# KwonGihyun/TweedieMix

Hardware: AMD Instinct MI355X
Metric: denoise steps/sec @ SDXL 1024^2 K=3 concepts (fusion phase); images/sec at 1/2/4/8 GPUs (higher is better)
Workload: dtype bf16

## Files before the change

include/tmix.h:

```cpp
#ifndef TMIX_H
#define TMIX_H

#include <stdint.h>

#ifdef __cplusplus
extern "C" {
#endif

#define TMIX_VERSION 100

enum { TMIX_OK = 0, TMIX_EINVAL = -1, TMIX_ESHAPE = -2, TMIX_EARCH = -3, TMIX_EALIGN = -4 };
enum { TMIX_F32 = 0, TMIX_F16 = 1, TMIX_BF16 = 2 };

int tmix_version(void);
const char* tmix_last_error_string(void);
int tmix_check_device(void);
void tmix_env_refresh(void);

int tmix_prof_begin(uint64_t* slots, int capacity, int detail);
int tmix_prof_end(void);

enum { TMIX_STEP_FUSION = 0, TMIX_STEP_PLAIN = 1, TMIX_STEP_RESAMPLE = 2 };
int tmix_fused_tweedie_step(const float* x, const void* eps, int eps_dtype, const float* masks,
                            float* out_x, float* out_x0, int K, int channels, int64_t hw, int mode,
                            float g, float sa, float s1, float sa_next, float s1_next, int is_last,
                            void* stream);
int tmix_fused_tweedie_step_dev(const float* x, const void* eps, int eps_dtype, const float* masks,
                                int64_t mask_seed_stride, float* out_x, float* out_x0, int K, int channels,
                                int64_t hw, int mode, int rows, int seeds, const float* params, void* stream);
int tmix_fused_tweedie_step_keep_dev(const float* x, const void* eps, int eps_dtype, const float* masks,
                                     int64_t mask_seed_stride, float* out_x, float* out_x0, int K, int channels,
                                     int64_t hw, int mode, int rows, int seeds, const float* params,
                                     const float* keep_x0, int64_t keep_x0_seed_stride, const float* keep_eps,
                                     int64_t keep_eps_seed_stride, const float* keep_w, int64_t keep_w_seed_stride, void* stream);
int tmix_step_prologue(const float* x, float* latent, float* t_dev, const float* params, int seeds, int rows,
                       int64_t n, void* stream);

int tmix_vpred_step(const void* x, const void* v, void* out, int dtype, int64_t n, float g,
                    float sa, float s1, float sa_next, float s1_next, void* stream);
int tmix_video_step_prologue(const float* x, float* x_u, int64_t clip_stride_u, float* t_u, float* x_c, int64_t clip_stride_c,
                             float* t_c, const float* params, int videos, int channels, int frames, int64_t hw, int row_channels,
                             void* stream);
int tmix_vpred_step_dev(float* x, const float* v_u, int64_t clip_stride_u, const float* v_c, int64_t clip_stride_c,
                        const float* params, int videos, int channels, int frames, int64_t hw, void* stream);
int tmix_frame_inject(void* x, int dtype, int clips, int frames, int64_t per_frame, int hard, float interp,
                      float one_minus_interp, void* stream);

enum { TMIX_EPI_NONE = 0, TMIX_EPI_GEGLU = 1, TMIX_EPI_F32OUT = 2 ,
       TMIX_EPI_GELU = 3 ,
       TMIX_EPI_QUICKGELU = 4  };
enum { TMIX_TILE_AUTO = 0, TMIX_TILE_128x128_S2 = 1, TMIX_TILE_256x128_S3 = 2, TMIX_TILE_128x128_S4 = 3,
       TMIX_TILE_256x256_S2 = 4, TMIX_TILE_256x128_W4 = 5, TMIX_TILE_256x256_W4 = 6, TMIX_TILE_128x160_S2 = 7,
       TMIX_TILE_128x160_S2_LW = 8, TMIX_TILE_256x128_S3_LW = 9, TMIX_TILE_128x128_S2_LW = 10, TMIX_TILE_256x256_S2_LW = 11,
       TMIX_TILE_128x160_S4 = 12 ,
       TMIX_TILE_64x160_W5 = 13 ,
       TMIX_TILE_256x320_S2 = 14 ,
       TMIX_TILE_32x160_W5 = 15 ,
       TMIX_TILE_256x256_PH = 16 ,
       TMIX_TILE_256x128_PH = 17,
       TMIX_TILE_128x160_S4_K2 = 18 ,
       TMIX_TILE_128x160_S3_LW = 19 ,
       TMIX_TILE_128x160_S4_LW2 = 20 ,
       TMIX_TILE_128x160_S4_LW4 = 21 ,
       TMIX_TILE_256x320_PH = 22 ,
       TMIX_TILE_128x160_W22 = 23 ,
       TMIX_TILE_CONV_HALO = 26 ,
       TMIX_TILE_COUNT = 26 };
typedef struct {
    const void* A;  int64_t lda, strideA;
    const void* W;  int64_t ldw, strideW;
    void*       C;  int64_t ldc, strideC;
    const float* bias;  int64_t strideBias;
    const void* residual; int64_t ldr, strideR;
    const float* rowgroup_bias;
    int32_t rows_per_group;
    void*   Ct; int64_t ldct, strideCt;
    int32_t n_trans_begin;
    int32_t M, N, K, batch;
    int32_t epilogue;
    int32_t tile_cfg;
    float* row_stats_out; int64_t strideStatsOut, ldStatsOut;
    const float* ln_stats; int64_t strideLnStats, ldLnStats;
    const float* ln_colsum; int64_t strideLnColsum;
    float ln_inv_c, ln_eps;
    int32_t ln_parts, reserved0;
    float* col_stats_out;
    int32_t w_period, reserved1;
} tmix_gemm_desc;
int tmix_gemm_bf16(const tmix_gemm_desc* d, void* stream);
int tmix_gemm_resolve_tile(const tmix_gemm_desc* d, int fp8_operands);
int tmix_gemm_f8copy_tile(int tile_cfg);
int tmix_gemm_prefetch_next(const void* next_weights, int64_t bytes, void* stream);
enum { TMIX_F8_A_BLOCK_SCALES = 1, TMIX_F8_GEGLU_OUT = 2, TMIX_F8_COPY_OUT = 4 };
#define TMIX_COLSTATS_ROWS 32
int tmix_gemm_fp8(const tmix_gemm_desc* d, const uint8_t* scale_a, const uint8_t* scale_w, void* stream);
int tmix_gemm_q_cross_attn(const tmix_gemm_desc* d, const void* K, int64_t ldk, int64_t strideK, const void* Vt, int64_t ldvt, int64_t strideVt,
                           void* O, int64_t ldo, int rows_per_image, int Skv, float scale, void* stream);
int tmix_quantize_fp8_rows(const void* X, int64_t ld, void* Q, int64_t ldq, uint8_t* scale_e8m0, int64_t rows, int K, void* stream);
int tmix_gemm_tile_shape(int tile_cfg, int* bm, int* bn);
int tmix_gemm_stats_parts(int N, int tile_cfg);

enum { TMIX_CONV_S1 = 0, TMIX_CONV_S2 = 1, TMIX_CONV_UP2 = 2, TMIX_CONV_T3 = 3, TMIX_CONV_S2A = 4 };
typedef struct {
    const void* X;
    const void* Wt;
    void*       Y;
    const float* bias;
    const float* batch_bias;
    const void* residual;
    int32_t B, H, W, Cin, Cout, mode;
    int32_t tile_cfg;
    int32_t batch_bias_images;
    float* col_stats_out;
    const void* S1; const void* S2;
    int32_t S1_channels, S2_channels;
} tmix_conv_desc;
int tmix_conv3x3_nhwc(const tmix_conv_desc* d, void* stream);
int tmix_conv3x3_nhwc_fp8(const tmix_conv_desc* d, const uint8_t* scale_x, const uint8_t* scale_w, void* stream);
int tmix_conv_resolve_tile(const tmix_conv_desc* d, int fp8_operands);

int tmix_conv_in(const float* x_nchw, const float* w_ohwi, const float* bias, void* y_nhwc,
                 int B, int Cin, int H, int W, int Cout, void* stream);
int tmix_conv_in_pre(const float* x_nchw, const float* w_ohwi, const float* bias, void* y_nhwc,
                     int B, int Cin, int H, int W, int Cout, const float* pre_w, const float* pre_b, void* stream);
int tmix_conv_out(const void* x_nhwc, const void* w_ohwi, const float* bias, float* y_nchw,
                  int B, int Cin, int H, int W, int Cout, void* stream);

int tmix_attn_fwd(const void* Q, int64_t ldq, int64_t strideQ, const void* K, int64_t ldk, int64_t strideK,
                  const void* Vt, int64_t ldvt, int64_t strideVt, void* O, int64_t ldo, int64_t strideO,
                  int B, int H, int Sq, int Skv, float scale, void* stream);
int tmix_attn_fwd_f8(const void* Q, int64_t ldq, int64_t strideQ, const void* K, int64_t ldk, int64_t strideK,
                     const void* Vt, int64_t ldvt, int64_t strideVt, void* O8, int64_t ldo8, void* scales, int64_t ldScale,
                     int B, int H, int Sq, int Skv, float scale, void* stream);
int64_t tmix_attn_split_ws_bytes(int B, int H, int Sq, int Skv);
int tmix_attn_fwd_ws(const void* Q, int64_t ldq, int64_t strideQ, const void* K, int64_t ldk, int64_t strideK,
                     const void* Vt, int64_t ldvt, int64_t strideVt, void* O, int64_t ldo, int64_t strideO,
                     int B, int H, int Sq, int Skv, float scale, void* ws, int64_t ws_bytes, void* stream);
int tmix_attn_fwd_f8_ws(const void* Q, int64_t ldq, int64_t strideQ, const void* K, int64_t ldk, int64_t strideK,
                        const void* Vt, int64_t ldvt, int64_t strideVt, void* O8, int64_t ldo8, void* scales, int64_t ldScale,
                        int B, int H, int Sq, int Skv, float scale, void* ws, int64_t ws_bytes, void* stream);

int64_t tmix_groupnorm_ws_floats(int B, int C, int groups);
int tmix_groupnorm_ws_chunks(int64_t HW);
int tmix_groupnorm_nhwc(const void* X1, int C1, const void* X2, int C2, void* Y, const float* gamma,
                        const float* beta, float* ws, int B, int64_t HW, int groups, float eps, int silu,
                        void* stream);
int tmix_groupnorm_nhwc_launches(int64_t HW, int C, int groups);
int tmix_groupnorm_nhwc_pre(const void* X1, int C1, const void* X2, int C2, void* Y, const float* gamma,
                            const float* beta, float* ws, int B, int64_t HW, int groups, float eps, int silu,
                            const float* cs1, int cs1_channels, const float* cs2, int cs2_channels, void* stream);
int tmix_groupnorm_nhwc_pre_f8(const void* X1, int C1, const void* X2, int C2, void* Y8, void* scales, const float* gamma,
                               const float* beta, float* ws, int B, int64_t HW, int groups, float eps, int silu,
                               const float* cs1, int cs1_channels, const float* cs2, int cs2_channels, void* stream);
int tmix_layernorm(const void* X, void* Y, const float* gamma, const float* beta, int64_t rows, int C,
                   float eps, void* stream);
int tmix_zero(void* ptr, int64_t nbytes, void* stream);
int tmix_concat_channels(const void* X1, int C1, const void* X2, int C2, void* Y, int64_t rows, void* stream);
int tmix_timestep_embedding(const float* values, float* out, int count, int dim, void* stream);
int tmix_softmax_rows(const float* S, int64_t ld_s, void* P, int64_t ld_p, int64_t rows, int cols, float scale, void* stream);
int tmix_softmax_rows_causal(const float* S, int64_t ld_s, void* P, int64_t ld_p, int64_t rows, int cols, float scale,
                             int seq, void* stream);
int tmix_softmax_rows_masked(const float* S, int64_t ld_s, void* P, int64_t ld_p, int64_t rows, int cols, int valid, float scale,
                             void* stream);
int tmix_temporal_attn(const void* QKV, int64_t ld, void* O, int64_t ldo, int clips, int frames, int64_t hw, int heads,
                       float scale, void* stream);
int tmix_lora_down(void* A, int64_t lda, int K, int64_t rows, const void* D, int P, int nsets, const float* dcolsum, const float* dbias,
                   float eps, const int* sets, int64_t rows_per_set, void* stream);
int tmix_affine_clamp(const float* x, float* y, int64_t n, float scale, float shift, float lo, float hi, void* stream);
int tmix_linear_small(const float* in, const void* W, const float* bias, const float* add, float* out,
                      int M, int N, int K, int act_in, int act_out, void* stream);
int tmix_linear_small_sections(const float* in, const void* W, const float* bias, float* out, int M, int N, int K,
                               int act_in, const int* sec_starts, int nsec, void* stream);

int tmix_conv3x3_f32(const float* x_nchw, const float* w_oihw, const float* bias, float* y_nchw, int B, int Cin, int H, int W, int Cout,
                     int stride, int silu, void* stream);
int tmix_adaptive_avgpool_f32(const float* x, float* y, int64_t planes, int H, int W, int OH, int OW, void* stream);
int tmix_linear_f32(const float* in, const float* W, const float* bias, float* out, int M, int N, int K, int act_in, int act_out, void* stream);
int tmix_i2v_temporal_encoder(const float* x, float* y, int clips, int frames, int channels, int64_t hw, const float* ln_gamma, const float* ln_beta,
                              const float* wq, const float* wk, const float* wv, const float* wo, const float* bo,
                              const float* w1, const float* b1, const float* w2, const float* b2, void* stream);

int tmix_xattn_token_maps(const void* Q, int64_t ldq, int64_t strideQ, const void* K, int64_t ldk, int64_t strideK, float* maps,
                          int B, int H, int Sq, int Lk, int row0, int row_step, int n_rows, const int32_t* tokens, int n_tok,
                          int accumulate, float scale, void* stream);

// ... 5 lines not shown
```

tweediemix_amd/csrc/gemm_conv.hip:

```cpp
#include "gemm_kernel.h"
#include "gemm_tilings.h"
#include <stdlib.h>

using namespace tmix_gemm;

namespace tmix_gemm {

bool f8_lockstep(int tile_cfg, int K, bool f8out) {
    return tile_cfg >= 1 && tile_cfg <= NUM_CFG && tile_has(tile_cfg, CAP_F8_LOCKSTEP) && K % 128 == 0 && !f8out;
}

int f8copy_tile(int tile_cfg) {
    if (tile_cfg < 1 || tile_cfg > NUM_CFG) TMIX_FAIL(TMIX_EINVAL, "gemm_f8copy_tile: tile_cfg=%d", tile_cfg);
    int cfg = TILINGS[tile_cfg].runs_as;
    while (!tile_has(cfg, CAP_F8C)) cfg = TILINGS[cfg].fb;
    return cfg;
}

#define TMIX_REFUSE(code, ...) do { tmix_set_error(__VA_ARGS__); return TileChoice{0, 0, (code)}; } while (0)

TileChoice resolve_tile(const TileTraits& t, int cfg) {
    const bool staged = t.n_trans_begin < 0 && (t.epilogue == TMIX_EPI_GEGLU ? (t.wide & 2) : (t.wide & 1));
    if (cfg <= 0 || cfg > NUM_CFG)
        cfg = (int64_t)((t.M + 255) / 256) * ((t.N + 127) / 128) * t.batch >= 192 ? 2 : 1;
// ... 144 lines not shown
        if (d->reserved0 & TMIX_F8_GEGLU_OUT) {
            if (d->epilogue != TMIX_EPI_GEGLU || !d->Ct || d->ldct < (int64_t)d->batch * d->M || (d->ldc % 8) || (d->strideC % 8) || (((uintptr_t)d->C) & 7))
                TMIX_FAIL(TMIX_EINVAL, "gemm_fp8: e4m3 GEGLU output needs the GEGLU epilogue, Ct = scale buffer [N/64][ldct >= batch*M] and 8-byte aligned C rows");
            p.f8out = 1; p.scale_out = (unsigned char*)d->Ct; p.ldScaleOut = d->ldct;
        }
    } else if (d->reserved0 & ~TMIX_F8_COPY_OUT) TMIX_FAIL(TMIX_EINVAL, "gemm: the fp8 operand flags in reserved0 belong to tmix_gemm_fp8");
    if (d->reserved0 & TMIX_F8_COPY_OUT) {
        if (has_trans || d->epilogue != TMIX_EPI_NONE || (d->reserved0 & TMIX_F8_GEGLU_OUT) || !d->Ct || (d->M % 32) || (d->N % 32) || (d->ldct % 8) || d->ldct < d->N
            || (((uintptr_t)d->Ct) & 7) || d->strideCt < (int64_t)d->batch * d->M * d->ldct)
            TMIX_FAIL(TMIX_EINVAL, "gemm: the e4m3 copy needs the plain bf16 epilogue, M %% 32 == 0, N %% 32 == 0, Ct = bytes [batch*M][ldct >= N, %% 8 == 0] and strideCt = byte offset of the scale array behind them");
        p.f8copy = (unsigned char*)d->Ct; p.ldF8copy = d->ldct;
        p.scale_out = (unsigned char*)d->Ct + d->strideCt; p.ldScaleOut = (int64_t)d->batch * d->M;
    }
    if (d->row_stats_out && (has_trans || d->epilogue != TMIX_EPI_NONE)) TMIX_FAIL(TMIX_EINVAL, "gemm: row_stats_out needs the plain bf16 epilogue");
    if (d->row_stats_out && (d->tile_cfg < 1 || d->tile_cfg > NUM_CFG || (((uintptr_t)d->row_stats_out) & 7) || (d->strideStatsOut & 1) || d->ldStatsOut < d->M))
        TMIX_FAIL(TMIX_EINVAL, "gemm: row_stats_out needs an explicit tile_cfg (its partial count depends on it) and 8-byte alignment");
    if (d->ln_stats && (!d->ln_colsum || !(d->ln_inv_c > 0.f) || d->ln_parts < 1 || d->ln_parts > 16 || (int64_t)d->ln_parts * d->ldLnStats * 8 >= (1ll << 31) || (((uintptr_t)d->ln_stats) & 7) || (d->strideLnStats & 1) || d->ldLnStats < d->M))
        TMIX_FAIL(TMIX_EINVAL, "gemm: fused LayerNorm needs ln_colsum, ln_inv_c > 0, 1 <= ln_parts <= 16 and 8-byte aligned ln_stats (< 2 GiB)");
    p.stats_out = d->row_stats_out; p.strideStatsOut = d->strideStatsOut; p.ldStatsOut = d->ldStatsOut;
    p.ln_stats = d->ln_stats; p.strideLnStats = d->strideLnStats; p.ldLnStats = d->ldLnStats; p.ln_parts = d->ln_parts;
    p.ln_colsum = d->ln_colsum; p.strideLnColsum = d->strideLnColsum; p.ln_inv_c = d->ln_inv_c; p.ln_eps = d->ln_eps;
    const bool c16 = d->C && aligned16(d->C) && (d->ldc % 8) == 0 && (d->strideC % 8) == 0;
    const bool r16 = !d->residual || (aligned16(d->residual) && (d->ldr % 8) == 0 && (d->strideR % 8) == 0);
    p.wide = 0;
    if (!tmix_env(TMIX_ENV_NARROW_EPILOGUE)) {
        if (d->epilogue == TMIX_EPI_GEGLU) { if (c16 || p.f8out) p.wide |= 2; }
        else if (d->epilogue == TMIX_EPI_F32OUT) { if (aligned16(d->C) && (d->ldc % 4) == 0 && (d->strideC % 4) == 0 && (d->N % 8) == 0) p.wide |= 1; }
        else if (c16 && r16 && (d->N % 8) == 0) p.wide |= 1;
        if (has_trans && aligned16(d->Ct) && (d->ldct % 8) == 0 && (d->strideCt % 8) == 0) p.wide |= 4;
    }
    if (d->col_stats_out) {
        if (fp8) TMIX_FAIL(TMIX_EINVAL, "gemm_fp8: col_stats_out is compiled for the bf16 tilings only (the fp8 loop would be remapped to a bf16 kernel over e4m3 bytes)");
        if (has_trans || d->epilogue != TMIX_EPI_NONE || d->row_stats_out || (d->reserved0 & TMIX_F8_COPY_OUT) || d->batch != 1 || (d->M % TMIX_COLSTATS_ROWS) || (d->N % 8)
            || !aligned16(d->col_stats_out) || !(p.wide & 1))
            TMIX_FAIL(TMIX_EINVAL, "gemm: col_stats_out needs the plain staged bf16 epilogue (16-byte aligned C / residual rows, N %% 8 == 0), batch == 1, M %% 32 == 0, "
                                   "and neither row_stats_out nor the e4m3 copy");
        p.cs_out = d->col_stats_out;
    }
    if (p.f8out && !(p.wide & 2)) TMIX_FAIL(TMIX_EINVAL, "gemm_fp8: e4m3 GEGLU output needs the staged epilogue");
    if (p.f8copy && !(p.wide & 1)) TMIX_FAIL(TMIX_EALIGN, "gemm: the e4m3 copy needs the staged epilogue (16-byte aligned C / residual rows, N %% 8 == 0)");
    if (fp8 && has_trans && !(p.wide & 4)) TMIX_FAIL(TMIX_EALIGN, "gemm_fp8: the transposed region needs a 16-byte aligned Ct with ldct %% 8 == 0");
    return TMIX_OK;
}

static int gemm_entry(const tmix_gemm_desc* d, bool fp8, const uint8_t* scaleA, const uint8_t* scaleW, void* stream, const QAExtra* qa = nullptr) {
    Params p;
    if (const int rc = gemm_params(d, fp8, scaleA, scaleW, qa != nullptr, p)) return rc;
    if (qa) return launch_qattn(p, *qa, d->batch, (hipStream_t)stream);
    return launch(0, p, d->batch, d->tile_cfg, (hipStream_t)stream);
}

alignas(16) static const uint8_t NO_SCALES[16] = {};

extern "C" int tmix_gemm_resolve_tile(const tmix_gemm_desc* d, int fp8_operands) {
    Params p;
    if (const int rc = gemm_params(d, fp8_operands != 0, fp8_operands ? NO_SCALES : nullptr, fp8_operands ? NO_SCALES : nullptr, false, p)) return rc;
    const TileChoice r = resolve_tile(traits_of(0, p, d->batch), d->tile_cfg);
    return r.err ? r.err : r.cfg;
}

extern "C" int tmix_gemm_q_cross_attn(const tmix_gemm_desc* d, const void* K, int64_t ldk, int64_t strideK, const void* Vt, int64_t ldvt, int64_t strideVt,
                                      void* O, int64_t ldo, int rows_per_image, int Skv, float scale, void* stream) {
    if (!d) TMIX_FAIL(TMIX_EINVAL, "gemm_q_cross_attn: null descriptor");
    if (d->reserved0 || d->residual || d->row_stats_out || d->col_stats_out || d->rowgroup_bias || d->epilogue != TMIX_EPI_NONE || (d->n_trans_begin >= 0 && d->n_trans_begin < d->N))
        TMIX_FAIL(TMIX_EINVAL, "gemm_q_cross_attn: the projection takes a bias and a folded LayerNorm only");
    const QAExtra x = {K, ldk, strideK, Vt, ldvt, strideVt, O, ldo, rows_per_image, Skv, scale};
    return gemm_entry(d, false, nullptr, nullptr, stream, &x);
}

extern "C" int tmix_gemm_bf16(const tmix_gemm_desc* d, void* stream) { return gemm_entry(d, false, nullptr, nullptr, stream); }

extern "C" int tmix_gemm_fp8(const tmix_gemm_desc* d, const uint8_t* scale_a, const uint8_t* scale_w, void* stream) {
    return gemm_entry(d, true, scale_a, scale_w, stream);
}

static int conv_params(const tmix_conv_desc* d, const uint8_t* scale_x, const uint8_t* scale_w, Params& p) {
    const bool fp8 = scale_x != nullptr;
    if (!d || !d->X || !d->Wt || !d->Y) TMIX_FAIL(TMIX_EINVAL, "conv3x3: null descriptor/operand");
    if (fp8 && (!scale_w || (d->Cin % 128) || d->S1 || d->S2 || (((uintptr_t)scale_x) & 3)))
        TMIX_FAIL(TMIX_EINVAL, "conv3x3_fp8: needs both scale arrays (scale_x 4-byte aligned), Cin %% 128 == 0 and no shortcut taps");
    if (d->B <= 0 || d->H <= 0 || d->W <= 0 || d->Cin <= 0 || d->Cout <= 0) TMIX_FAIL(TMIX_ESHAPE, "conv3x3: empty problem");
    if (d->Cin % BK) TMIX_FAIL(TMIX_ESHAPE, "conv3x3: Cin=%d must be a multiple of %d", d->Cin, BK);
    if (d->Cout % 4) TMIX_FAIL(TMIX_ESHAPE, "conv3x3: Cout=%d must be a multiple of 4", d->Cout);
    if (d->mode < TMIX_CONV_S1 || d->mode > TMIX_CONV_S2A) TMIX_FAIL(TMIX_EINVAL, "conv3x3: bad mode %d", d->mode);
    if ((d->mode == TMIX_CONV_S2 || d->mode == TMIX_CONV_S2A) && ((d->H | d->W) & 1)) TMIX_FAIL(TMIX_ESHAPE, "conv3x3: stride-2 needs even H,W");
    if (!aligned16(d->X) || !aligned16(d->Wt) || (((uintptr_t)d->Y) & 7)) TMIX_FAIL(TMIX_EALIGN, "conv3x3: pointer alignment");
    if ((d->bias && (((uintptr_t)d->bias) & 15)) || (d->batch_bias && (((uintptr_t)d->batch_bias) & 15))) TMIX_FAIL(TMIX_EALIGN, "conv3x3: bias alignment");
    p = {};
    p.H = d->H; p.Wd = d->W; p.Cin = d->Cin; p.mode = d->mode;
    p.ntaps = d->mode == TMIX_CONV_T3 ? 3 : 9;
    const bool half = d->mode == TMIX_CONV_S2 || d->mode == TMIX_CONV_S2A;
    p.Ho = half ? d->H / 2 : (d->mode == TMIX_CONV_UP2 ? d->H * 2 : d->H);
    p.Wo = half ? d->W / 2 : (d->mode == TMIX_CONV_UP2 ? d->W * 2 : d->W);
    const int64_t M = (int64_t)d->B * p.Ho * p.Wo;
    if (M > 0x7fffffff / 4) TMIX_FAIL(TMIX_ESHAPE, "conv3x3: too many output pixels");
    if ((int64_t)d->B * d->H * d->W * d->Cin >= (1ll << 30) || (int64_t)d->Cout * 9 * d->Cin >= (1ll << 30)) TMIX_FAIL(TMIX_ESHAPE, "conv3x3: operand larger than 2 GiB");
    p.A = (const bf16_t*)d->X;
    p.W = (const bf16_t*)d->Wt; p.ldw = p.ntaps * (int64_t)d->Cin;
    p.C = (bf16_t*)d->Y; p.ldc = d->Cout;
    p.bias = d->bias;
    p.R = (const bf16_t*)d->residual; p.ldr = d->Cout;
    p.rgb = d->batch_bias; p.rows_per_group = p.Ho * p.Wo * (d->batch_bias_images > 1 ? d->batch_bias_images : 1);
    p.n_trans_begin = -1;
    p.M = (int)M; p.N = d->Cout; p.K = p.ntaps * d->Cin;
    if (d->S1 || d->S2) {
        const int c1 = d->S1_channels, c2 = d->S2 ? d->S2_channels : 0;
        if (!d->S1 || d->mode != TMIX_CONV_S1 || c1 <= 0 || (c1 % BK) || c2 < 0 || (c2 % BK) || (d->S2 && c2 == 0) || !aligned16(d->S1) || (d->S2 && !aligned16(d->S2)) || d->residual)
            TMIX_FAIL(TMIX_EINVAL, "conv3x3: shortcut taps need the stride-1 mode, S1 (S2 only with S1), channel counts that are multiples of %d, 16-byte alignment and no residual", BK);
        if ((int64_t)d->B * d->H * d->W * (c1 > c2 ? c1 : c2) >= (1ll << 30) || (int64_t)d->Cout * (9ll * d->Cin + c1 + c2) >= (1ll << 30)) TMIX_FAIL(TMIX_ESHAPE, "conv3x3: shortcut operand larger than 2 GiB");
        p.S1 = (const bf16_t*)d->S1; p.S2 = (const bf16_t*)d->S2; p.c1s = c1; p.c2s = c2;
        p.bytesS1 = (unsigned)((int64_t)d->B * d->H * d->W * c1 * 2); p.bytesS2 = (unsigned)((int64_t)d->B * d->H * d->W * c2 * 2);
        p.K += c1 + c2;
        p.ldw = p.K;
    }
    p.epilogue = TMIX_EPI_NONE;
    p.bytesA = (unsigned)((int64_t)d->B * d->H * d->W * d->Cin * (fp8 ? 1 : 2));
    p.bytesW = (unsigned)((int64_t)d->Cout * p.K * (fp8 ? 1 : 2));
    if (fp8) { p.scaleA = scale_x; p.scaleW = scale_w; p.ldScaleA = d->Cin / 32; }
    p.wide = (!tmix_env(TMIX_ENV_NARROW_EPILOGUE) && aligned16(d->Y) && (d->Cout % 8) == 0 && (!d->residual || aligned16(d->residual))) ? 1 : 0;
    if (p.S1 && !p.wide) TMIX_FAIL(TMIX_EALIGN, "conv3x3: shortcut taps need the staged epilogue (16-byte aligned Y, Cout %% 8 == 0)");
    if (d->col_stats_out) {
        if ((M % TMIX_COLSTATS_ROWS) || !aligned16(d->col_stats_out) || !p.wide)
            TMIX_FAIL(TMIX_EINVAL, "conv3x3: col_stats_out needs B*Ho*Wo %% 32 == 0, Cout %% 8 == 0 and 16-byte aligned Y / residual");
        p.cs_out = d->col_stats_out;
    }
    return TMIX_OK;
}

static int conv_entry(const tmix_conv_desc* d, const uint8_t* scale_x, const uint8_t* scale_w, void* stream) {
    Params p;
    if (const int rc = conv_params(d, scale_x, scale_w, p)) return rc;
    return launch(1, p, 1, d->tile_cfg, (hipStream_t)stream);
}

extern "C" int tmix_conv_resolve_tile(const tmix_conv_desc* d, int fp8_operands) {
    Params p;
    if (const int rc = conv_params(d, fp8_operands ? NO_SCALES : nullptr, fp8_operands ? NO_SCALES : nullptr, p)) return rc;
    const TileChoice r = resolve_tile(traits_of(1, p, 1), d->tile_cfg);
    return r.err ? r.err : r.cfg;
}

extern "C" int tmix_conv3x3_nhwc(const tmix_conv_desc* d, void* stream) { return conv_entry(d, nullptr, nullptr, stream); }

extern "C" int tmix_conv3x3_nhwc_fp8(const tmix_conv_desc* d, const uint8_t* scale_x, const uint8_t* scale_w, void* stream) {
    if (!scale_x) TMIX_FAIL(TMIX_EINVAL, "conv3x3_fp8: null scale array");
    return conv_entry(d, scale_x, scale_w, stream);
}
```

tweediemix_amd/csrc/gemm_kernel.h:

```cpp
#pragma once
#include "common.h"
#include <type_traits>
#include <stdlib.h>

namespace tmix_gemm {

#ifndef TMIX_ABL
#define TMIX_ABL 0
#endif
constexpr int ABL = TMIX_ABL;

constexpr int BK = 64;
typedef __attribute__((ext_vector_type(8))) __bf16 frag_ab;

static __device__ __forceinline__ float xor32_sum(float x) {
    auto r = __builtin_amdgcn_permlane32_swap(__float_as_uint(x), __float_as_uint(x), false, false);
    return __uint_as_float(r[0]) + __uint_as_float(r[1]);
}

static __device__ __forceinline__ float quad_max(float x) {
    float y = __int_as_float(__builtin_amdgcn_update_dpp(0, __float_as_int(x), 0xB1, 0xf, 0xf, false));
    x = fmaxf(x, y);
    y = __int_as_float(__builtin_amdgcn_update_dpp(0, __float_as_int(x), 0x4E, 0xf, 0xf, false));
    return fmaxf(x, y);
}

template <int CTRL> static __device__ __forceinline__ float dpp_row(float x) {
    return __int_as_float(__builtin_amdgcn_update_dpp(0, __float_as_int(x), CTRL, 0xf, 0xf, false));
}
static __device__ __forceinline__ float swap32_sum(float a, float b) {
    auto r = __builtin_amdgcn_permlane32_swap(__float_as_uint(a), __float_as_uint(b), false, false);
    return __uint_as_float(r[0]) + __uint_as_float(r[1]);
}
static __device__ __forceinline__ float swap16_sum(float a, float b) {
    auto r = __builtin_amdgcn_permlane16_swap(__float_as_uint(a), __float_as_uint(b), false, false);
    return __uint_as_float(r[0]) + __uint_as_float(r[1]);
}

struct Params {
    const bf16_t* A; int64_t lda, strideA;
    const bf16_t* W; int64_t ldw, strideW;
    bf16_t* C; int64_t ldc, strideC;
    const float* bias; int64_t strideBias;
    const bf16_t* R; int64_t ldr, strideR;
    const float* rgb; int rows_per_group;
    bf16_t* Ct; int64_t ldct, strideCt; int n_trans_begin;
    int M, N, K, tiles_m, tiles_n, group_m, epilogue;
    unsigned bytesA, bytesW;
    float* stats_out; int64_t strideStatsOut, ldStatsOut;
    const float* ln_stats; int64_t strideLnStats, ldLnStats; const float* ln_colsum; int64_t strideLnColsum;
    float ln_inv_c, ln_eps; int ln_parts;
    int H, Wd, Cin, Ho, Wo, mode, ntaps;
    unsigned long long* prof; int prof_detail;
    int wide;
    const unsigned char* scaleA; const unsigned char* scaleW; int64_t strideScaleA, strideScaleW;
    int64_t ldScaleA;
    unsigned char* scale_out; int64_t ldScaleOut; int f8out;
    unsigned char* f8copy; int64_t ldF8copy;
    const char* pf; long long pf_bytes;
    int pf_per;
    int w_period, w_groups; unsigned w_magic;
    float* cs_out;
    const bf16_t* S1; const bf16_t* S2; int c1s, c2s; unsigned bytesS1, bytesS2;
};

static __device__ __forceinline__ void blds16(__amdgpu_buffer_rsrc_t rsrc, unsigned voff, unsigned soff, char* lds_dst) {
    __builtin_amdgcn_raw_ptr_buffer_load_lds(rsrc, (__attribute__((address_space(3))) void*)lds_dst, 16, voff, soff, 0, 0);
}

constexpr int f8_block_cap(int bn) { return bn >= 256 ? 88 : 224; }

template <int N> static __device__ __forceinline__ void wait_vmcnt() { asm volatile("s_waitcnt vmcnt(%0)" ::"n"(N) : "memory"); }

template <int BM, int BN, int WM, int WN, int NS, int CONV, int LW = 0, int PH = 0, int KS = 1, int CS = 0, int EK = 0, int SC = 0>
__global__ void __launch_bounds__((WM * WN * KS + LW) * 64, LW ? (NS * (BM + BN) * 128 > 80 * 1024 ? 2 : 3) : (KS == 1 && WM * WN == 4 && NS * (BM + BN) * 128 > 80 * 1024) ? 1 : 2)
gemm_conv_kernel(const Params p) {
    constexpr bool PHL = PH >= 1 && PH <= 3;
    static_assert(!PHL || (WM * WN == 8 && !LW && !CONV && NS == 4 && BM % 128 == 0 && BN % 32 == 0 && (BM / WM) % 32 == 0 && (BN / WN) % 32 == 0), "phase-offset mainloop geometry");
    static_assert(PH <= 3 || KS == 1, "fp8 lock-step loop: no in-workgroup split-K");
    static_assert(!(CONV && PH >= 4) || (PH == 5 && !SC && BM % ((LW ? LW : WM * WN)) == 0 && BM / (LW ? LW : WM * WN) <= 64), "fp8 convolution geometry");
    static_assert(KS == 1 || (KS == 2 && !LW && !PH && !CONV), "in-workgroup split-K geometry");
    static_assert(!SC || (CONV && (LW == 0 || LW == 2)), "shortcut taps belong to the convolution (lock-step tilings, with or without two loader waves)");
    constexpr bool F8C = !CONV && (LW ? (PH >= 4 && EK == 4) : true) && (BM / WM / 32) * (BN / WN / 32) <= 8;
    constexpr bool F8 = PH >= 2;
    constexpr bool F8B = PH == 3 || PH == 5;
    constexpr bool F8L = PH >= 4;
    constexpr int SCP = (F8L && F8B) ? 1 : 0;
    constexpr int EB = F8 ? 1 : 2;
    constexpr int NW = WM * WN;
    constexpr int TM = BM / WM, TN = BN / WN;
    constexpr int FM = TM / 32, FN = TN / 32;
    constexpr int A_TILE = BM * 128, B_TILE = BN * 128, STAGE = A_TILE + B_TILE + SCP * 1024;
    static_assert(!SCP || 4 * BM <= 1024, "scale piece");
    constexpr int SLOT = (BM + BN) * 64;
    constexpr int RING = PHL ? 4 * SLOT : NS * STAGE;
    constexpr int SW = LW ? LW : NW * KS;
    constexpr int IA = BM / 8, IB = BN / 8;
    constexpr int RA = (IA + SW - 1) / SW, RB = (IB + SW - 1) / SW;
    constexpr int L = RA + RB + SCP;
    static_assert(RA >= 1 && RB >= 1 && FM >= 1 && FN >= 1, "tile/wave geometry");
    static_assert(PHL || (NS - 2) * L <= 63, "vmcnt immediate");

    extern __shared__ __attribute__((aligned(16))) char smem[];
#ifndef TMIX_NO_KERNARG_TOUCH
    kernarg_touch<(int)sizeof(Params)>();
#endif
    const int tid = threadIdx.x;
    const int lane = tid & 63;
    const int w = __builtin_amdgcn_readfirstlane(tid >> 6);
    const int kg = KS > 1 ? w / NW : 0;
    const int wm_ = KS > 1 ? w - kg * NW : w;
    const int wr = wm_ / WN, wc = wm_ - wr * WN;
    const bool prof_on = p.prof != nullptr && tid == 0;
    unsigned long long pt0 = 0, pt1 = 0, pt2 = 0;
    if (prof_on) pt0 = prof_enter(p.prof, (blockIdx.x | blockIdx.y) == 0, p.prof_detail);
    constexpr int PFU = 8;
    unsigned pf_keep[PFU];
#pragma unroll
    for (int u = 0; u < PFU; ++u) pf_keep[u] = 0;
    if (p.pf && (!LW || w >= WM * WN)) {
        const long long nwg = (long long)gridDim.x * gridDim.y, nth = (LW ? LW : WM * WN * KS) * 64;
        const long long lines = (p.pf_bytes + 127) >> 7; const int per = p.pf_per;
        const long long first = ((long long)blockIdx.y * gridDim.x + blockIdx.x) * nth + (LW ? tid - WM * WN * 64 : tid);
#pragma unroll
        for (int u = 0; u < PFU; ++u) {
            const long long ln = first + (long long)u * nwg * nth;
            if (u < per && ln < lines) asm volatile("global_load_dword %0, %1, off" : "=v"(pf_keep[u]) : "v"(p.pf + (ln << 7)) : "memory");
        }
    }
    const bool loader = LW && (w >= NW);
    const bool stager = LW ? loader : true;
    const int sw_id = LW ? max(w - NW, 0) : w;

#ifdef TMIX_XCD_X_ONLY
    const int bid = xcd_remap(blockIdx.x, gridDim.x), by = blockIdx.y;
#else
    int bid, by;
    xcd_remap_grid(bid, by);
#endif
    const int per_group = p.group_m * p.tiles_n;
    const int grp = bid / per_group;
    const int first_m = grp * p.group_m;
    const int gsize = min(p.tiles_m - first_m, p.group_m);
    const int rem = bid - grp * per_group;
    const int tile_n = rem / gsize, tile_m = first_m + (rem - tile_n * gsize);
    const int m0 = tile_m * BM, n0 = tile_n * BN;
    const int m0l = (ABL & 1) ? 0 : m0, n0l = (ABL & 1) ? 0 : n0;
    const int bzw = p.w_period > 0 ? (int)__umulhi((unsigned)by, p.w_magic) : by;
    const int bz = p.w_period > 0 ? (by - bzw * p.w_groups) * p.w_period + bzw : by;

    const bf16_t* Ab = (const bf16_t*)((const char*)p.A + (int64_t)bz * p.strideA * EB);
    const bf16_t* Wb = (const bf16_t*)((const char*)p.W + (int64_t)bzw * p.strideW * EB);
    const __amdgpu_buffer_rsrc_t rsA = __builtin_amdgcn_make_buffer_rsrc((void*)Ab, 0, p.bytesA, 0x00020000);
    const __amdgpu_buffer_rsrc_t rsW = __builtin_amdgcn_make_buffer_rsrc((void*)Wb, 0, p.bytesW, 0x00020000);

    const int lrow = lane >> 3;
    auto slot_a = [&](int r) { int i = r * SW + sw_id; if constexpr (IA % SW != 0) i = min(i, IA - 1); return i; };
    auto slot_w = [&](int r) { int i = r * SW + sw_id; if constexpr (IB % SW != 0) i = min(i, IB - 1); return i; };
    constexpr int RAa = (LW && !CONV) ? 1 : RA, RBa = LW ? 1 : RB;
    unsigned woff[RBa], aoff[RAa];
    int asw[(CONV && !LW) ? RA : 1];
    unsigned cbase[CONV ? RA : 1], cmask[CONV ? RA : 1];
    int cpix[(CONV && SC) ? RA : 1];
    auto conv_row = [&](int r, int m, unsigned swb) __attribute__((always_inline)) {
        if constexpr (CONV) {
            const int hw = p.Ho * p.Wo;
            const int b = m / hw, rem = m - b * hw;
            const int py = rem / p.Wo, px = rem - py * p.Wo;
            int iy0, ix0; unsigned par = 0;
            if (p.mode == TMIX_CONV_S1 || p.mode == TMIX_CONV_T3) { iy0 = py - 1; ix0 = px - 1; }
            else if (p.mode == TMIX_CONV_S2) { iy0 = 2 * py - 1; ix0 = 2 * px - 1; }
            else if (p.mode == TMIX_CONV_S2A) { iy0 = 2 * py; ix0 = 2 * px; }
            else { iy0 = (py - 1) >> 1; ix0 = (px - 1) >> 1; par = (unsigned)((py - 1) & 1) << 16 | (unsigned)((px - 1) & 1) << 17; }
            unsigned mk = 0;
#pragma unroll
            for (int t = 0; t < 9; ++t) {
                if (t >= p.ntaps) break;
                const int ky = p.mode == TMIX_CONV_T3 ? t : t / 3, kx = p.mode == TMIX_CONV_T3 ? 1 : t - (t / 3) * 3;
                bool ok;
                if (p.mode == TMIX_CONV_UP2) { const int uy = py + ky - 1, ux = px + kx - 1; ok = (uy >= 0) & (uy < 2 * p.H) & (ux >= 0) & (ux < 2 * p.Wd); }
                else { const int iy = iy0 + ky, ix = ix0 + kx; ok = (iy >= 0) & (iy < p.H) & (ix >= 0) & (ix < p.Wd); }
                mk |= (unsigned)ok << t;
            }
            cbase[r] = (unsigned)(((b * p.H + iy0) * p.Wd + ix0) * p.Cin) * (unsigned)EB + swb;
            cmask[r] = mk | par;
            if constexpr (SC) cpix[r] = (b * p.H + py) * p.Wd + px;
        }
    };
    unsigned aoffp[2], amaxp[2], woffp[2], wmaxp[2], swp[2];
    if constexpr (LW) {
        if (loader) {
#pragma unroll
            for (int pp = 0; pp < 2; ++pp) {
                const int par = (LW >= 2) ? (sw_id & 1) : pp;
                const unsigned sw = ((lane & 7) ^ ((4 * par + (lane >> 4)) & 7)) * 8;
                swp[pp] = sw;
                woffp[pp] = (unsigned)(n0l + par * 8 + lrow) * (unsigned)p.ldw * (unsigned)EB + sw * 2u;
                wmaxp[pp] = (unsigned)(p.N - 1) * (unsigned)p.ldw * (unsigned)EB + sw * 2u;
                aoffp[pp] = (unsigned)(m0l + par * 8 + lrow) * (unsigned)p.lda * (unsigned)EB + sw * 2u;
                amaxp[pp] = (unsigned)(p.M - 1) * (unsigned)p.lda * (unsigned)EB + sw * 2u;
            }
            if constexpr (CONV) {
#pragma unroll
                for (int r = 0; r < RA; ++r) {
                    int m = m0l + slot_a(r) * 8 + lrow; if (m > p.M - 1) m = p.M - 1;
                    conv_row(r, m, swp[r & 1] * 2u);
                }
            }
        }
    } else
    if (stager && !PHL) {
#pragma unroll
    for (int r = 0; r < RB; ++r) {
        const int idx = slot_w(r);
        const int sw = ((lane & 7) ^ ((4 * idx + (lane >> 4)) & 7)) * 8;
        int n = n0l + idx * 8 + lrow; if (n > p.N - 1) n = p.N - 1;
        woff[r] = (unsigned)n * (unsigned)p.ldw * (unsigned)EB + (unsigned)sw * 2u;
    }
#pragma unroll
    for (int r = 0; r < RA; ++r) {
        const int idx = slot_a(r);
        const int sw = ((lane & 7) ^ ((4 * idx + (lane >> 4)) & 7)) * 8;
        int m = m0l + idx * 8 + lrow; if (m > p.M - 1) m = p.M - 1;
        asw[r] = sw;
        if constexpr (CONV) {
            conv_row(r, m, (unsigned)sw * 2u);
            aoff[r] = 0;
        } else {
            aoff[r] = (unsigned)m * (unsigned)p.lda * (unsigned)EB + (unsigned)sw * 2u;
        }
    }
    }

    constexpr int PA = PHL ? BM / 16 / NW : 1, PB = PHL ? (BN / 16 + NW - 1) / NW : 1;
    auto ph_w = [&](int r) { int i = r * NW + w; if constexpr ((BN / 16) % NW != 0) i = min(i, BN / 16 - 1); return i; };
    unsigned phA[PA], phW[PB];
    if constexpr (PHL) {
        const unsigned ch = (unsigned)(((lane & 3) ^ ((lane >> 4) & 3)) * (16 / EB));
#pragma unroll
        for (int r = 0; r < PA; ++r) {
            int m = m0l + (r * NW + w) * 16 + (lane >> 2); if (m > p.M - 1) m = p.M - 1;
            phA[r] = ((unsigned)m * (unsigned)p.lda + ch) * (unsigned)EB;
        }
#pragma unroll
        for (int r = 0; r < PB; ++r) {
            int n = n0l + ph_w(r) * 16 + (lane >> 2); if (n > p.N - 1) n = p.N - 1;
            phW[r] = ((unsigned)n * (unsigned)p.ldw + ch) * (unsigned)EB;
        }
    }
    auto ph_stage = [&](int slot, int s) {
        char* sA = smem + slot * SLOT;
        char* sW = sA + BM * 64;
#pragma unroll
        for (int r = 0; r < PA; ++r) blds16(rsA, phA[r], (unsigned)s * 64u, sA + (r * NW + w) * 1024);
#pragma unroll
        for (int r = 0; r < PB; ++r) blds16(rsW, phW[r], (unsigned)s * 64u, sW + ph_w(r) * 1024);
    };

    const int nk = p.K / (F8L ? 2 * BK : BK);
    int tap = 0, cc = 0;
    int cpt = CONV ? p.Cin / (F8L ? 2 * BK : BK) : 1;
    const int ntaps_all = SC ? p.ntaps + (p.c1s > 0) + (p.c2s > 0) : p.ntaps;

    unsigned cvo[RA];
    constexpr int SRW = (CONV && SCP) ? BM / SW : 1;
    int sb_ = 0, sy_ = 0, sx_ = 0; unsigned scv = 0x80000000u;
    if constexpr (CONV && SCP) {
        if (stager) {
            const int hw = p.Ho * p.Wo;
            int m = m0l + sw_id * SRW + min(lane, SRW - 1); if (m > p.M - 1) m = p.M - 1;
            sb_ = m / hw; const int rem = m - sb_ * hw;
            sy_ = rem / p.Wo; sx_ = rem - sy_ * p.Wo;
        }
    }
    auto conv_tap_offsets = [&]() __attribute__((always_inline)) {
        if constexpr (SC) {
            if (tap >= p.ntaps) {
                const int Cs = tap == p.ntaps ? p.c1s : p.c2s;
#pragma unroll
                for (int r = 0; r < RA; ++r)
                    cvo[r] = (unsigned)(cpix[r] * Cs + (LW ? (int)swp[r & 1] : asw[LW ? 0 : r])) * 2u;
                cpt = Cs / BK;
                return;
            }
        }
        const int ky = p.mode == TMIX_CONV_T3 ? tap : tap / 3, kx = p.mode == TMIX_CONV_T3 ? 1 : tap - ky * 3;
        const unsigned pixb = (unsigned)p.Cin * (unsigned)EB, rowb = (unsigned)p.Wd * pixb;
        if (p.mode == TMIX_CONV_UP2) {
            const unsigned sd = (ky == 2 ? rowb : 0u) + (kx == 2 ? pixb : 0u), ay = ky == 1 ? rowb : 0u, ax = kx == 1 ? pixb : 0u;
#pragma unroll
            for (int r = 0; r < RA; ++r) {
                const unsigned o = cbase[r] + sd + ((cmask[r] >> 16) & 1u) * ay + ((cmask[r] >> 17) & 1u) * ax;
                cvo[r] = ((cmask[r] >> tap) & 1u) ? o : 0x80000000u;
            }
        } else {
            const unsigned sd = (unsigned)ky * rowb + (unsigned)kx * pixb;
#pragma unroll
            for (int r = 0; r < RA; ++r) cvo[r] = ((cmask[r] >> tap) & 1u) ? cbase[r] + sd : 0x80000000u;
        }
        if constexpr (CONV && SCP) {
            int iy, ix; bool ok;
            if (p.mode == TMIX_CONV_S1 || p.mode == TMIX_CONV_T3) { iy = sy_ + ky - 1;     ix = sx_ + kx - 1;     ok = (iy >= 0) & (iy < p.H) & (ix >= 0) & (ix < p.Wd); }
            else if (p.mode == TMIX_CONV_S2) { iy = 2 * sy_ + ky - 1; ix = 2 * sx_ + kx - 1; ok = (iy >= 0) & (iy < p.H) & (ix >= 0) & (ix < p.Wd); }
            else if (p.mode == TMIX_CONV_S2A) { iy = 2 * sy_ + ky; ix = 2 * sx_ + kx; ok = (iy < p.H) & (ix < p.Wd); }
            else { const int uy = sy_ + ky - 1, ux = sx_ + kx - 1;
                   ok = (uy >= 0) & (uy < 2 * p.H) & (ux >= 0) & (ux < 2 * p.Wd); iy = uy >> 1; ix = ux >> 1; }
            scv = ok ? (unsigned)((sb_ * p.H + iy) * p.Wd + ix) * (unsigned)(p.Cin / 32) : 0x80000000u;
        }
    };
    if constexpr (CONV) { if (stager) conv_tap_offsets(); }

    const bool sc_mine = SCP && (CONV ? lane < SRW : (lane % SW == sw_id) && (16 * lane < 4 * BM));
    unsigned sc_voff = 0;
    __amdgpu_buffer_rsrc_t rsSc = rsA;
    if constexpr (SCP) {
        if constexpr (CONV) rsSc = __builtin_amdgcn_make_buffer_rsrc((void*)p.scaleA, 0, (int)(p.bytesA / 32), 0x00020000);
        else {
            rsSc = __builtin_amdgcn_make_buffer_rsrc((void*)p.scaleA, 0, (int)((int64_t)(p.K / 32) * p.ldScaleA), 0x00020000);
            sc_voff = (unsigned)((16 * lane) / BM) * (unsigned)p.ldScaleA + (unsigned)((16 * lane) % BM) + (unsigned)(bz * p.strideScaleA + m0l);
        }
    }
    auto scale_piece = [&](char* sA, int kt) __attribute__((always_inline)) {
        if constexpr (SCP && CONV) {
            if (sc_mine) __builtin_amdgcn_raw_ptr_buffer_load_lds(rsSc, (__attribute__((address_space(3))) void*)(sA + A_TILE + B_TILE + sw_id * SRW * 4), 4, scv, (unsigned)cc * 4u, 0, 0);
        } else if constexpr (SCP) { if (sc_mine) blds16(rsSc, sc_voff, (unsigned)kt * 4u * (unsigned)p.ldScaleA, sA + A_TILE + B_TILE); }
    };
    auto dma_piece = [&](const int r, char* sA, int kt) __attribute__((always_inline)) {
        if constexpr (!CONV && !LW) {
            if (r < RA) blds16(rsA, aoff[r], (unsigned)kt * (BK * 2), sA + slot_a(r) * 1024);
            else if (r < RA + RB) blds16(rsW, woff[r - RA], (unsigned)kt * (BK * 2), sA + A_TILE + slot_w(r - RA) * 1024);
            else scale_piece(sA, kt);
        }
    };
    auto stage = [&](int buf, int kt) __attribute__((always_inline)) {
        char* sA = smem + buf * STAGE;
        char* sW = sA + A_TILE;
        bool a_done = false;
        unsigned wk = (unsigned)kt * (BK * 2);
#ifndef TMIX_ABL_WSEQ
        if constexpr (CONV && !LW) {
            const int tap_u = __builtin_amdgcn_readfirstlane(tap), cc_u = __builtin_amdgcn_readfirstlane(cc);
            if (SC && tap_u >= p.ntaps) wk = (unsigned)(p.ntaps * p.Cin + (tap_u > p.ntaps ? p.c1s : 0)) * 2u + (unsigned)cc_u * (BK * 2);
            else wk = (unsigned)(tap_u * p.Cin) * (unsigned)EB + (unsigned)cc_u * (BK * 2);
        }
#endif
        if constexpr (CONV && SC) {
            const int tap_u = __builtin_amdgcn_readfirstlane(tap);
            const void* base = tap_u < p.ntaps ? (const void*)Ab : (tap_u == p.ntaps ? (const void*)p.S1 : (const void*)p.S2);
            const unsigned bytes = tap_u < p.ntaps ? p.bytesA : (tap_u == p.ntaps ? p.bytesS1 : p.bytesS2);
            const __amdgpu_buffer_rsrc_t rs = __builtin_amdgcn_make_buffer_rsrc((void*)base, 0, bytes, 0x00020000);
            a_done = true;
#pragma unroll
            for (int r = 0; r < RA; ++r) blds16(rs, cvo[r], (unsigned)cc * (BK * 2), sA + slot_a(r) * 1024);
        }
        if (!a_done)
#pragma unroll
        for (int r = 0; r < RA; ++r) {
            if constexpr (CONV) blds16(rsA, cvo[r], (unsigned)cc * (BK * 2), sA + slot_a(r) * 1024);
            else if constexpr (LW) blds16(rsA, min(aoffp[(r * LW) & 1] + (unsigned)(slot_a(r) >> 1) * (unsigned)(16 * EB * p.lda), amaxp[(r * LW) & 1]),
                                          (unsigned)kt * (BK * 2), sA + slot_a(r) * 1024);
            else                blds16(rsA, aoff[r], (unsigned)kt * (BK * 2), sA + slot_a(r) * 1024);
        }
#pragma unroll
        for (int r = 0; r < RB; ++r) {
            if constexpr (LW) blds16(rsW, min(woffp[(r * LW) & 1] + (unsigned)(slot_w(r) >> 1) * (unsigned)(16 * EB * p.ldw), wmaxp[(r * LW) & 1]),
                                     wk, sW + slot_w(r) * 1024);
            else              blds16(rsW, woff[r], wk, sW + slot_w(r) * 1024);
        }
        scale_piece(sA, kt);
// ... 481 lines not shown
                    if (m + 8 <= p.M) *(uint4*)dst = v;
                    else {
                        const unsigned u[4] = {v.x, v.y, v.z, v.w};
                        for (int k = 0; k < 8 && m + k < p.M; ++k) dst[k] = (bf16_t)(u[k >> 1] >> ((k & 1) * 16));
                    }
                }
            }
            if (prof_on) prof_leave(p.prof, p.prof_detail, pt0, pt1, pt2);
            return;
        }
        if constexpr (SQ) {
            bf16_t* Ct = p.Ct + (int64_t)bz * p.strideCt;
            if (EK == 3 || (p.wide & 4)) {
                constexpr int CF = (FN % 2 == 0) ? 2 : 1, SR = CF * 64 + 16, LPR = CF * 4, RPI = 64 / LPR, NP = 32 / RPI;
                char* stg = smem + w * STG_MAX;
                const int rr = lane / LPR, cc = (lane % LPR) * 8;
#pragma unroll
                for (int i = 0; i < FM; ++i) {
                    const int nl = n0 + wc * TN + i * 32 + l31;
                    const float bv = (bias && nl < p.N) ? bias[nl] : 0.f;
#pragma unroll
                    for (int c = 0; c < FN / CF; ++c) {
#pragma unroll
                        for (int jj = 0; jj < CF; ++jj)
#pragma unroll
                            for (int g = 0; g < 4; ++g) {
                                const int j = c * CF + jj, ml = wr * TM + j * 32 + g * 8 + lhi * 4;
                                const float4 rs = p.ln_stats ? *(const float4*)(ln_rs + ml) : make_float4(1.f, 1.f, 1.f, 1.f);
                                uint2 v;
                                v.x = pack_bf2(fmaf(acc[i][j][g * 4 + 0], rs.x, bv), fmaf(acc[i][j][g * 4 + 1], rs.y, bv));
                                v.y = pack_bf2(fmaf(acc[i][j][g * 4 + 2], rs.z, bv), fmaf(acc[i][j][g * 4 + 3], rs.w, bv));
                                *(uint2*)(stg + l31 * SR + (jj * 32 + g * 8 + lhi * 4) * 2) = v;
                            }
#pragma unroll
                        for (int ps = 0; ps < NP; ++ps) {
                            const int r = ps * RPI + rr, n = n0 + wc * TN + i * 32 + r, m = m0 + wr * TM + c * CF * 32 + cc;
                            const uint4 v = *(const uint4*)(stg + r * SR + cc * 2);
                            if (n >= p.N || m >= p.M) continue;
                            bf16_t* dst = Ct + (int64_t)(n - p.n_trans_begin) * p.ldct + m;
                            if (m + 8 <= p.M) *(uint4*)dst = v;
                            else {
                                const unsigned u[4] = {v.x, v.y, v.z, v.w};
                                for (int k = 0; k < 8 && m + k < p.M; ++k) dst[k] = (bf16_t)(u[k >> 1] >> ((k & 1) * 16));
                            }
                        }
                    }
                }
                if (prof_on) prof_leave(p.prof, p.prof_detail, pt0, pt1, pt2);
                return;
            }
#pragma unroll
            for (int i = 0; i < FM; ++i) {
                const int n = n0 + wc * TN + i * 32 + l31;
                if (n >= p.N) continue;
                const float bv = bias ? bias[n] : 0.f;
                bf16_t* row = Ct + (int64_t)(n - p.n_trans_begin) * p.ldct;
#pragma unroll
                for (int j = 0; j < FN; ++j)
#pragma unroll
                    for (int g = 0; g < 4; ++g) {
                        const int ml = wr * TM + j * 32 + g * 8 + lhi * 4, m = m0 + ml;
                        if (m >= p.M) continue;
                        const float4 rs = p.ln_stats ? *(const float4*)(ln_rs + ml) : make_float4(1.f, 1.f, 1.f, 1.f);
                        const float o0 = fmaf(acc[i][j][g * 4 + 0], rs.x, bv), o1 = fmaf(acc[i][j][g * 4 + 1], rs.y, bv);
                        const float o2 = fmaf(acc[i][j][g * 4 + 2], rs.z, bv), o3 = fmaf(acc[i][j][g * 4 + 3], rs.w, bv);
                        if (m + 3 < p.M && ((p.ldct & 3) == 0)) {
                            uint2 v;
                            v.x = pack_bf2(o0, o1);
                            v.y = pack_bf2(o2, o3);
                            *(uint2*)(row + m) = v;
                        } else {
                            const float o[4] = {o0, o1, o2, o3};
#pragma unroll
                            for (int r = 0; r < 4; ++r) if (m + r < p.M) row[m + r] = f2bf(o[r]);
                        }
                    }
            }
        }
        if (prof_on) prof_leave(p.prof, p.prof_detail, pt0, pt1, pt2);
        return;
    }

    bf16_t* Cb = p.C + (int64_t)bz * p.strideC;
    if (EK == 1 || (EK == 0 && p.epilogue == TMIX_EPI_GEGLU)) {
        if (EK == 1 || (p.wide & 2)) {
            char* stg = smem + w * STG_MAX;
            auto chunk = [&](int i, int j0, auto cf_tag) {
                constexpr int CF = decltype(cf_tag)::value, OC = CF * 16, SR = OC * 2 + 16, LPR = OC / 8, RPI = 64 / LPR, NP = 32 / RPI;
                const int rr = lane / LPR, cc = (lane % LPR) * 8;
#pragma unroll
                for (int jj = 0; jj < CF; ++jj) {
                    const int j = j0 + jj;
#pragma unroll
                    for (int g = 0; g < 2; ++g) {
                        float o[4];
                        const float4 ba = *(const float4*)(bias_lds + wc * TN + j * 32 + g * 8 + lhi * 4), bg = *(const float4*)(bias_lds + wc * TN + j * 32 + g * 8 + lhi * 4 + 16);
                        const float bav[4] = {ba.x, ba.y, ba.z, ba.w}, bgv[4] = {bg.x, bg.y, bg.z, bg.w};
#pragma unroll
                        for (int r = 0; r < 4; ++r) {
                            const float a = fmaf(acc[i][j][g * 4 + r], rs_row[i], bav[r]), gt = fmaf(acc[i][j][(g + 2) * 4 + r], rs_row[i], bgv[r]);
                            o[r] = a * gelu_erf_f(gt);
                        }
                        uint2 v; v.x = pack_bf2(o[0], o[1]); v.y = pack_bf2(o[2], o[3]);
                        *(uint2*)(stg + l31 * SR + (jj * 16 + g * 8 + lhi * 4) * 2) = v;
                    }
                }
#pragma unroll
                for (int ps = 0; ps < NP; ++ps) {
                    const int r = ps * RPI + rr, m = m0 + wr * TM + i * 32 + r;
                    const uint4 v = *(const uint4*)(stg + r * SR + cc * 2);
                    const int nb = n0 + wc * TN + (j0 + cc / 16) * 32;
                    const int col = (n0 + wc * TN) / 2 + j0 * 16 + cc;
                    if constexpr (CF >= 2) {
                        if (p.f8out) {
                            const unsigned u[4] = {v.x, v.y, v.z, v.w};
                            float f[8], am = 0.f;
#pragma unroll
                            for (int k = 0; k < 4; ++k) { f[2 * k] = __uint_as_float(u[k] << 16); f[2 * k + 1] = __uint_as_float(u[k] & 0xffff0000u);
                                                          am = fmaxf(am, fmaxf(fabsf(f[2 * k]), fabsf(f[2 * k + 1]))); }
                            am = quad_max(am);
                            const int e = e8m0_for_amax(am);
                            const float inv = exp2_neg_int(e);
                            int q0 = __builtin_amdgcn_cvt_pk_fp8_f32(f[0] * inv, f[1] * inv, 0, false); q0 = __builtin_amdgcn_cvt_pk_fp8_f32(f[2] * inv, f[3] * inv, q0, true);
                            int q1 = __builtin_amdgcn_cvt_pk_fp8_f32(f[4] * inv, f[5] * inv, 0, false); q1 = __builtin_amdgcn_cvt_pk_fp8_f32(f[6] * inv, f[7] * inv, q1, true);
                            if (m >= p.M || nb >= p.N) continue;
                            *(uint2*)((unsigned char*)p.C + (int64_t)bz * p.strideC + (int64_t)m * p.ldc + col) = make_uint2((unsigned)q0, (unsigned)q1);
                            if ((lane & 3) == 0) p.scale_out[(int64_t)(col >> 5) * p.ldScaleOut + (int64_t)bz * p.M + m] = (unsigned char)(e + 127);
                            continue;
                        }
                    }
                    if (m >= p.M || nb >= p.N) continue;
                    *(uint4*)(Cb + (int64_t)m * p.ldc + col) = v;
                }
            };
#pragma unroll
            for (int i = 0; i < FM; ++i) {
                constexpr int C4 = FN / 4, R4 = FN % 4;
#pragma unroll
                for (int c = 0; c < C4; ++c) chunk(i, c * 4, std::integral_constant<int, 4>{});
                if constexpr (R4 >= 2) chunk(i, C4 * 4, std::integral_constant<int, 2>{});
                if constexpr (R4 & 1) chunk(i, FN - 1, std::integral_constant<int, 1>{});
            }
            if (prof_on) prof_leave(p.prof, p.prof_detail, pt0, pt1, pt2);
            return;
        }
#pragma unroll
        for (int i = 0; i < FM; ++i) {
            const int m = m0 + wr * TM + i * 32 + l31;
            if (m >= p.M) continue;
#pragma unroll
            for (int j = 0; j < FN; ++j) {
                const int nb = n0 + wc * TN + j * 32;
                if (nb >= p.N) continue;
#pragma unroll
                for (int g = 0; g < 2; ++g) {
                    const int nv = nb + g * 8 + lhi * 4;
                    float o[4];
#pragma unroll
                    for (int r = 0; r < 4; ++r) {
                        float a = acc[i][j][g * 4 + r], gt = acc[i][j][(g + 2) * 4 + r];
                        if (bias) { a = fmaf(a, rs_row[i], bias[nv + r]); gt = fmaf(gt, rs_row[i], bias[nv + 16 + r]); }
                        else { a *= rs_row[i]; gt *= rs_row[i]; }
                        o[r] = a * gelu_erf_f(gt);
                    }
                    uint2 v; v.x = pack_bf2(o[0], o[1]); v.y = pack_bf2(o[2], o[3]);
                    *(uint2*)(Cb + (int64_t)m * p.ldc + nb / 2 + g * 8 + lhi * 4) = v;
// ... 12 lines not shown
#pragma unroll
        for (int i = 0; i < FM; ++i) {
#pragma unroll
            for (int q = 0; q < 4; ++q) { sa1[i][q] = 0.f; sa2[i][q] = 0.f; }
            sb1[i][0] = sb1[i][1] = sb2[i][0] = sb2[i][1] = 0.f;
        }
        auto cs_flush = [&](float (&cv)[16], int mb, int nc, bool ncok, auto cf_tag) __attribute__((always_inline)) {
            constexpr int CF = decltype(cf_tag)::value;
            float t[8], u[4];
#pragma unroll
            for (int k = 0; k < 8; ++k) t[k] = swap32_sum(cv[k], cv[8 + k]);
#pragma unroll
            for (int k = 0; k < 4; ++k) u[k] = swap16_sum(t[k], t[k + 4]);
#pragma unroll
            for (int k = 0; k < 4; ++k) u[k] += dpp_row<0x128>(u[k]);
            if constexpr (CF == 1) {
#pragma unroll
                for (int k = 0; k < 4; ++k) u[k] += dpp_row<0x124>(u[k]);
            }
            if (!(lane & (CF == 1 ? 12 : 8)) && mb < p.M && ncok)
                *(float4*)(p.cs_out + ((int64_t)(mb >> 5) * 2 + (lane >> 5)) * p.N + nc + ((lane >> 4) & 1) * 4) = make_float4(u[0], u[1], u[2], u[3]);
        };
        auto cs_add = [&](float (&cv)[16], const uint4& v) __attribute__((always_inline)) {
            const unsigned u[4] = {v.x, v.y, v.z, v.w};
#pragma unroll
            for (int k = 0; k < 4; ++k) {
                const float lo = __uint_as_float(u[k] << 16), hi = __uint_as_float(u[k] & 0xffff0000u);
                cv[2 * k] += lo; cv[2 * k + 1] += hi;
                cv[8 + 2 * k] = fmaf(lo, lo, cv[8 + 2 * k]); cv[9 + 2 * k] = fmaf(hi, hi, cv[9 + 2 * k]);
            }
        };
        auto chunk = [&](int j0, auto cf_tag, auto fl_tag) __attribute__((always_inline)) {
            constexpr int CF = decltype(cf_tag)::value, CW = CF * 32, SR = CW * 4 + 16, LPR = CW / 8, RPI = 64 / LPR, NP = 32 / RPI;
            constexpr int FL = decltype(fl_tag)::value;
            const int rr = lane / LPR, cc = (lane % LPR) * 8;
            const int nc = n0 + wc * TN + j0 * 32 + cc;
            const bool ncok = nc < p.N;
            if constexpr ((FL & 1) != 0) {
                constexpr int CI = CF == 2 ? 0 : (FN / 2) * 4;
                const bool lnf = p.ln_stats != nullptr;
                const float4 bq0 = *(const float4*)(bias_lds + wc * TN + j0 * 32 + cc), bq1 = *(const float4*)(bias_lds + wc * TN + j0 * 32 + cc + 4);
                const float bq[8] = {bq0.x, bq0.y, bq0.z, bq0.w, bq1.x, bq1.y, bq1.z, bq1.w};
                float tq[8];
                if constexpr (CONV) {
                    const float4 t0 = *(const float4*)(rgb_lds + wc * TN + j0 * 32 + cc), t1 = *(const float4*)(rgb_lds + wc * TN + j0 * 32 + cc + 4);
                    tq[0] = t0.x; tq[1] = t0.y; tq[2] = t0.z; tq[3] = t0.w; tq[4] = t1.x; tq[5] = t1.y; tq[6] = t1.z; tq[7] = t1.w;
                }
#pragma unroll
                for (int i = 0; i < FM; ++i) {
                    const int mb = m0 + wr * TM + i * 32;
                    float cv[(FL & 8) ? 16 : 1];
                    if constexpr ((FL & 8) != 0) {
#pragma unroll
                        for (int k = 0; k < 16; ++k) cv[k] = 0.f;
                    }
#pragma unroll
                    for (int jj = 0; jj < CF; ++jj)
#pragma unroll
                        for (int g = 0; g < 4; ++g)
                            *(float4*)(stg + l31 * SR + (jj * 32 + g * 8 + lhi * 4) * 4) =
                                make_float4(acc[i][j0 + jj][g * 4 + 0], acc[i][j0 + jj][g * 4 + 1], acc[i][j0 + jj][g * 4 + 2], acc[i][j0 + jj][g * 4 + 3]);
#pragma unroll
                    for (int ps = 0; ps < NP; ++ps) {
                        const int r = ps * RPI + rr, m = mb + r;
                        const float4 v0 = *(const float4*)(stg + r * SR + cc * 4), v1 = *(const float4*)(stg + r * SR + cc * 4 + 16);
                        const float rsl = ln_rs[wr * TM + i * 32 + r];
                        const float rs = lnf ? rsl : 1.f;
                        float o[8] = {v0.x, v0.y, v0.z, v0.w, v1.x, v1.y, v1.z, v1.w};
#pragma unroll
                        for (int k = 0; k < 8; ++k) o[k] = fmaf(o[k], rs, bq[k]);
                        if constexpr (CONV) {
#pragma unroll
                            for (int k = 0; k < 8; ++k) o[k] += tq[k];
                        }
                        if constexpr (WPREF) {
                            const uint4 rq = rw[i * WP_I + CI + (CF == 2 ? (j0 / 2) * 4 : 0) + ps];
                            const unsigned ru[4] = {rq.x, rq.y, rq.z, rq.w};
#pragma unroll
                            for (int k = 0; k < 4; ++k) { o[2 * k] += __uint_as_float(ru[k] << 16); o[2 * k + 1] += __uint_as_float(ru[k] & 0xffff0000u); }
                        }
                        uint4 v;
                        v.x = pack_bf2(o[0], o[1]); v.y = pack_bf2(o[2], o[3]); v.z = pack_bf2(o[4], o[5]); v.w = pack_bf2(o[6], o[7]);
                        const bool ok = m < p.M && ncok;
                        if (ok) *(uint4*)(Cb + (int64_t)m * p.ldc + nc) = v;
                        if constexpr (F8C && (FL & 4) != 0) {
                            const unsigned u8[4] = {v.x, v.y, v.z, v.w};
                            float f[8], am = 0.f;
#pragma unroll
                            for (int k = 0; k < 4; ++k) { f[2 * k] = __uint_as_float(u8[k] << 16); f[2 * k + 1] = __uint_as_float(u8[k] & 0xffff0000u);
                                                          am = fmaxf(am, fmaxf(fabsf(f[2 * k]), fabsf(f[2 * k + 1]))); }
                            am = quad_max(am);
                            const int e = e8m0_for_amax(am);
                            const float inv = exp2_neg_int(e);
                            int q0 = __builtin_amdgcn_cvt_pk_fp8_f32(f[0] * inv, f[1] * inv, 0, false); q0 = __builtin_amdgcn_cvt_pk_fp8_f32(f[2] * inv, f[3] * inv, q0, true);
                            int q1 = __builtin_amdgcn_cvt_pk_fp8_f32(f[4] * inv, f[5] * inv, 0, false); q1 = __builtin_amdgcn_cvt_pk_fp8_f32(f[6] * inv, f[7] * inv, q1, true);
                            if (ok) {
                                *(uint2*)(p.f8copy + ((int64_t)bz * p.M + m) * p.ldF8copy + nc) = make_uint2((unsigned)q0, (unsigned)q1);
                                if ((lane & 3) == 0) p.scale_out[(int64_t)(nc >> 5) * p.ldScaleOut + (int64_t)bz * p.M + m] = (unsigned char)(e + 127);
                            }
                        }
                        if constexpr ((FL & 2) != 0) {
                            const unsigned u[4] = {v.x, v.y, v.z, v.w};
                            float a1 = 0.f, a2 = 0.f;
#pragma unroll
                            for (int k = 0; k < 4; ++k) {
                                const float lo = __uint_as_float(u[k] << 16), hi = __uint_as_float(u[k] & 0xffff0000u);
                                a1 += lo + hi; a2 = fmaf(lo, lo, a2); a2 = fmaf(hi, hi, a2);
                            }
                            if (!ok) { a1 = 0.f; a2 = 0.f; }
                            if constexpr (CF == 2) { sa1[i][ps] += a1; sa2[i][ps] += a2; } else { sb1[i][ps] += a1; sb2[i][ps] += a2; }
                        }
                        if constexpr ((FL & 8) != 0) cs_add(cv, v);
                    }
                    if constexpr ((FL & 8) != 0) cs_flush(cv, mb, nc, ncok, cf_tag);
                }
                return;
            }
            float bv[8];
#pragma unroll
            for (int k = 0; k < 8; ++k) bv[k] = 0.f;
            if (bias && ncok && !(ABL & 16)) {
                const float4 b0 = *(const float4*)(bias + nc), b1 = *(const float4*)(bias + nc + 4);
                bv[0] = b0.x; bv[1] = b0.y; bv[2] = b0.z; bv[3] = b0.w; bv[4] = b1.x; bv[5] = b1.y; bv[6] = b1.z; bv[7] = b1.w;
            }
#pragma unroll
            for (int i = 0; i < FM; ++i) {
                const int mb = m0 + wr * TM + i * 32;
                float cv[(FL & 8) ? 16 : 1];
                if constexpr ((FL & 8) != 0) {
#pragma unroll
                    for (int k = 0; k < 16; ++k) cv[k] = 0.f;
                }
                uint4 rv[NP];
                if (Rb && !(ABL & 64)) {
#pragma unroll
                    for (int ps = 0; ps < NP; ++ps) {
                        const int m = mb + ps * RPI + rr;
                        if constexpr (WPREF) rv[ps] = rw[i * WP_I + (CF == 2 ? (j0 / 2) * 4 : (FN / 2) * 4) + ps];
                        else if (m < p.M && ncok) rv[ps] = *(const uint4*)(Rb + (int64_t)m * p.ldr + nc);
                    }
                }
#pragma unroll
                for (int jj = 0; jj < CF; ++jj)
#pragma unroll
                    for (int g = 0; g < 4; ++g)
                        *(float4*)(stg + l31 * SR + (jj * 32 + g * 8 + lhi * 4) * 4) =
                            make_float4(acc[i][j0 + jj][g * 4 + 0], acc[i][j0 + jj][g * 4 + 1], acc[i][j0 + jj][g * 4 + 2], acc[i][j0 + jj][g * 4 + 3]);
#pragma unroll
                for (int ps = 0; ps < NP; ++ps) {
                    const int r = ps * RPI + rr, m = mb + r;
                    const float4 v0 = *(const float4*)(stg + r * SR + cc * 4), v1 = *(const float4*)(stg + r * SR + cc * 4 + 16);
                    if (m >= p.M || !ncok) continue;
                    float o[8] = {v0.x, v0.y, v0.z, v0.w, v1.x, v1.y, v1.z, v1.w};
                    if (bias) { const float rs = p.ln_stats ? ln_rs[wr * TM + i * 32 + r] : 1.f;
#pragma unroll
                                for (int k = 0; k < 8; ++k) o[k] = fmaf(o[k], rs, bv[k]); }
                    else if (p.ln_stats) { const float rs = ln_rs[wr * TM + i * 32 + r];
#pragma unroll
                                for (int k = 0; k < 8; ++k) o[k] *= rs; }
                    if (p.rgb) {
                        const float* rg = p.rgb + (int64_t)(m / p.rows_per_group) * p.N + nc;
                        const float4 b0 = *(const float4*)rg, b1 = *(const float4*)(rg + 4);
                        o[0] += b0.x; o[1] += b0.y; o[2] += b0.z; o[3] += b0.w; o[4] += b1.x; o[5] += b1.y; o[6] += b1.z; o[7] += b1.w;
                    }
                    if (p.epilogue == TMIX_EPI_GELU) {
#pragma unroll
                        for (int k = 0; k < 8; ++k) o[k] = gelu_erf_f(o[k]);
                    } else if (p.epilogue == TMIX_EPI_QUICKGELU) {
#pragma unroll
                        for (int k = 0; k < 8; ++k) o[k] = o[k] * __builtin_amdgcn_rcpf(1.0f + __builtin_amdgcn_exp2f(-2.4554669595930157f * o[k]));
                    }
                    if (Rb && !(ABL & 64)) {
                        const unsigned u[4] = {rv[ps].x, rv[ps].y, rv[ps].z, rv[ps].w};
#pragma unroll
                        for (int k = 0; k < 4; ++k) { o[2 * k] += bf2f((bf16_t)(u[k] & 0xffff)); o[2 * k + 1] += bf2f((bf16_t)(u[k] >> 16)); }
                    }
                    if (f32out) {
                        float* dst = (float*)p.C + (int64_t)bz * p.strideC + (int64_t)m * p.ldc + nc;
                        *(float4*)dst = make_float4(o[0], o[1], o[2], o[3]);
                        *(float4*)(dst + 4) = make_float4(o[4], o[5], o[6], o[7]);
                    } else {
                        uint4 v;
                        v.x = pack_bf2(o[0], o[1]); v.y = pack_bf2(o[2], o[3]); v.z = pack_bf2(o[4], o[5]); v.w = pack_bf2(o[6], o[7]);
                        if constexpr (ABL & 32) asm volatile("" :: "v"(v.x), "v"(v.y), "v"(v.z), "v"(v.w));
                        else *(uint4*)(Cb + (int64_t)m * p.ldc + nc) = v;
                        if constexpr (F8C) if (p.f8copy) {
                            const unsigned u8[4] = {v.x, v.y, v.z, v.w};
                            float f[8], am = 0.f;
#pragma unroll
                            for (int k = 0; k < 4; ++k) { f[2 * k] = __uint_as_float(u8[k] << 16); f[2 * k + 1] = __uint_as_float(u8[k] & 0xffff0000u);
                                                          am = fmaxf(am, fmaxf(fabsf(f[2 * k]), fabsf(f[2 * k + 1]))); }
                            am = quad_max(am);
                            const int e = e8m0_for_amax(am);
                            const float inv = exp2_neg_int(e);
                            int q0 = __builtin_amdgcn_cvt_pk_fp8_f32(f[0] * inv, f[1] * inv, 0, false); q0 = __builtin_amdgcn_cvt_pk_fp8_f32(f[2] * inv, f[3] * inv, q0, true);
                            int q1 = __builtin_amdgcn_cvt_pk_fp8_f32(f[4] * inv, f[5] * inv, 0, false); q1 = __builtin_amdgcn_cvt_pk_fp8_f32(f[6] * inv, f[7] * inv, q1, true);
                            *(uint2*)(p.f8copy + ((int64_t)bz * p.M + m) * p.ldF8copy + nc) = make_uint2((unsigned)q0, (unsigned)q1);
                            if ((lane & 3) == 0) p.scale_out[(int64_t)(nc >> 5) * p.ldScaleOut + (int64_t)bz * p.M + m] = (unsigned char)(e + 127);
                        }
                        if (sto) {
                            const unsigned u[4] = {v.x, v.y, v.z, v.w};
                            float a1 = 0.f, a2 = 0.f;
#pragma unroll
                            for (int k = 0; k < 4; ++k) {
                                const float lo = __uint_as_float(u[k] << 16), hi = __uint_as_float(u[k] & 0xffff0000u);
                                a1 += lo + hi; a2 = fmaf(lo, lo, a2); a2 = fmaf(hi, hi, a2);
                            }
                            if constexpr (CF == 2) { sa1[i][ps] += a1; sa2[i][ps] += a2; } else { sb1[i][ps] += a1; sb2[i][ps] += a2; }
                        }
                        if constexpr ((FL & 8) != 0) cs_add(cv, v);
                    }
                }
                if constexpr ((FL & 8) != 0) cs_flush(cv, mb, nc, ncok, cf_tag);
            }
        };
        constexpr int C2 = FN / 2;
        auto chunks = [&](auto fl_tag) __attribute__((always_inline)) {
#pragma unroll
            for (int c = 0; c < C2; ++c) chunk(c * 2, std::integral_constant<int, 2>{}, fl_tag);
            if constexpr (FN & 1) chunk(FN - 1, std::integral_constant<int, 1>{}, fl_tag);
        };
        const bool fastp = (WPREF || !Rb) && !f32out && p.epilogue == TMIX_EPI_NONE && (!p.rgb || (CONV && rgb_one)) && !(ABL & 0xf0);
        bool f8q = false;
        if constexpr (F8C) f8q = p.f8copy != nullptr;
        if constexpr (EK == 4) { if constexpr (F8C) { if (!sto) chunks(std::integral_constant<int, 5>{}); else chunks(std::integral_constant<int, 7>{}); } }
        else if constexpr (CS) { if (!fastp) chunks(std::integral_constant<int, 8>{}); else chunks(std::integral_constant<int, 9>{}); }
        else if (!fastp) chunks(std::integral_constant<int, 0>{});
        else if (!f8q) { if (!sto) chunks(std::integral_constant<int, 1>{}); else chunks(std::integral_constant<int, 3>{}); }
        else { if constexpr (F8C) { if (!sto) chunks(std::integral_constant<int, 5>{}); else chunks(std::integral_constant<int, 7>{}); } }
        if (sto) {
#pragma unroll
            for (int i = 0; i < FM; ++i) {
                if constexpr (C2 > 0) {
#pragma unroll
                    for (int q = 0; q < 4; ++q) {
                        float a1 = sa1[i][q], a2 = sa2[i][q];
#pragma unroll
                        for (int off = 1; off < 8; off <<= 1) { a1 += __shfl_xor(a1, off); a2 += __shfl_xor(a2, off); }
                        if ((lane & 7) == 0) redw[wc * BM + wr * TM + i * 32 + q * 8 + (lane >> 3)] = make_float2(a1, a2);
                    }
                }
                if constexpr (FN & 1) {
#pragma unroll
                    for (int q = 0; q < 2; ++q) {
                        float b1 = sb1[i][q], b2 = sb2[i][q];
#pragma unroll
                        for (int off = 1; off < 4; off <<= 1) { b1 += __shfl_xor(b1, off); b2 += __shfl_xor(b2, off); }
                        if ((lane & 3) == 0) {
                            float2* dst = redw + wc * BM + wr * TM + i * 32 + q * 16 + (lane >> 2);
                            if constexpr (C2 > 0) { const float2 t = *dst; *dst = make_float2(t.x + b1, t.y + b2); }
                            else *dst = make_float2(b1, b2);
                        }
                    }
                }
            }
            __syncthreads();
            if (tid < BM && m0 + tid < p.M) {
                float2 t = redw[tid];
#pragma unroll
                for (int c = 1; c < WN; ++c) { const float2 u = redw[c * BM + tid]; t.x += u.x; t.y += u.y; }
                sto[(int64_t)tile_n * p.ldStatsOut + m0 + tid] = t;
            }
        }
        if (prof_on) prof_leave(p.prof, p.prof_detail, pt0, pt1, pt2);
        return;
    }
    float2* red = (float2*)smem;
#pragma unroll
    for (int i = 0; i < FM; ++i) {
        const int m = m0 + wr * TM + i * 32 + l31;
        float s1 = 0.f, s2 = 0.f;
        if (m < p.M) {
        const float* rg = p.rgb ? p.rgb + (int64_t)(m / p.rows_per_group) * p.N : nullptr;
#pragma unroll
        for (int j = 0; j < FN; ++j)
#pragma unroll
            for (int g = 0; g < 4; ++g) {
                const int n = n0 + wc * TN + j * 32 + g * 8 + lhi * 4;
                if (n >= p.N) continue;
                float o[4];
#pragma unroll
                for (int r = 0; r < 4; ++r) o[r] = acc[i][j][g * 4 + r];
                if (bias) { const float4 b4 = *(const float4*)(bias + n);
                            o[0] = fmaf(o[0], rs_row[i], b4.x); o[1] = fmaf(o[1], rs_row[i], b4.y);
                            o[2] = fmaf(o[2], rs_row[i], b4.z); o[3] = fmaf(o[3], rs_row[i], b4.w); }
                else if (p.ln_stats) { o[0] *= rs_row[i]; o[1] *= rs_row[i]; o[2] *= rs_row[i]; o[3] *= rs_row[i]; }
                if (rg)   { const float4 b4 = *(const float4*)(rg + n);   o[0] += b4.x; o[1] += b4.y; o[2] += b4.z; o[3] += b4.w; }
                if (p.epilogue == TMIX_EPI_GELU) {
#pragma unroll
                    for (int r = 0; r < 4; ++r) o[r] = gelu_erf_f(o[r]);
                } else if (p.epilogue == TMIX_EPI_QUICKGELU) {
#pragma unroll
                    for (int r = 0; r < 4; ++r) o[r] = o[r] * __builtin_amdgcn_rcpf(1.0f + __builtin_amdgcn_exp2f(-2.4554669595930157f * o[r]));
                }
                if (Rb) {
                    uint2 rv;
                    if constexpr (PREF) rv = rres[i][j][g];
                    else rv = *(const uint2*)(Rb + (int64_t)m * p.ldr + n);
                    o[0] += bf2f((bf16_t)(rv.x & 0xffff)); o[1] += bf2f((bf16_t)(rv.x >> 16));
                    o[2] += bf2f((bf16_t)(rv.y & 0xffff)); o[3] += bf2f((bf16_t)(rv.y >> 16));
                }
                if (p.epilogue == TMIX_EPI_F32OUT) {
                    *(float4*)((float*)p.C + (int64_t)bz * p.strideC + (int64_t)m * p.ldc + n) = make_float4(o[0], o[1], o[2], o[3]);
                } else {
                    uint2 v; v.x = pack_bf2(o[0], o[1]); v.y = pack_bf2(o[2], o[3]);
                    *(uint2*)(Cb + (int64_t)m * p.ldc + n) = v;
                    if (sto) {
                        const float r0 = __uint_as_float(v.x << 16), r1 = __uint_as_float(v.x & 0xffff0000u);
                        const float r2 = __uint_as_float(v.y << 16), r3 = __uint_as_float(v.y & 0xffff0000u);
                        s1 += (r0 + r1) + (r2 + r3);
                        s2 = fmaf(r0, r0, s2); s2 = fmaf(r1, r1, s2); s2 = fmaf(r2, r2, s2); s2 = fmaf(r3, r3, s2);
                    }
                }
            }
        }
        if (sto) {
            s1 = xor32_sum(s1); s2 = xor32_sum(s2);
            if (!lhi) red[wc * BM + wr * TM + i * 32 + l31] = make_float2(s1, s2);
        }
    }
    if (sto) {
        __syncthreads();
        if (tid < BM && m0 + tid < p.M) {
            float2 t = red[tid];
#pragma unroll
            for (int c = 1; c < WN; ++c) { const float2 u = red[c * BM + tid]; t.x += u.x; t.y += u.y; }
            sto[(int64_t)tile_n * p.ldStatsOut + m0 + tid] = t;
        }
    }
    if (prof_on) prof_leave(p.prof, p.prof_detail, pt0, pt1, pt2);
}

template <int BM, int BN, int WM, int WN, int NS, int CONV, int LW = 0, int PH = 0, int KS = 1, int CS = 0, int EK = 0, int SC = 0>
int launch_cfg(Params& p, int batch, hipStream_t st) {
    static_assert(KS == 1 || BM * BN * 4 <= NS * (BM + BN) * 128, "the split-K hand-over must fit in the staging ring");
    constexpr int SMEM = ((PH >= 1 && PH <= 3) ? 4 * (BM + BN) * 64 : NS * ((BM + BN) * 128 + (PH == 5 ? 1024 : 0))) + (BM + BN) * 16 + BM * 4 + BN * 4 + (CONV ? BN * 4 : 0)
                       + (PH == 3 ? BM * f8_block_cap(BN) : 0);
    static_assert(SMEM <= 160 * 1024, "LDS");
    static bool attr_set = false;
    auto kern = gemm_conv_kernel<BM, BN, WM, WN, NS, CONV, LW, PH, KS, CS, EK, SC>;
    if (!attr_set) {
        hipError_t e = hipFuncSetAttribute((const void*)kern, hipFuncAttributeMaxDynamicSharedMemorySize, SMEM);
        if (e != hipSuccess) TMIX_FAIL((int)e, "hipFuncSetAttribute: %s", hipGetErrorString(e));
        attr_set = true;
    }
    p.tiles_m = (p.M + BM - 1) / BM; p.tiles_n = (p.N + BN - 1) / BN;
    p.group_m = BM >= 256 ? 4 : 8;
    if (BM >= 256 && BN >= 256) p.group_m = 8;
    if ((int64_t)p.tiles_m * p.tiles_n * batch > 0x7fffffffLL) TMIX_FAIL(TMIX_ESHAPE, "gemm: %lld x %d workgroups exceed the 32-bit linear grid id", (long long)p.tiles_m * p.tiles_n, batch);
    dim3 grid(p.tiles_m * p.tiles_n, batch, 1);
    p.prof = tmix_prof_take(&p.prof_detail);
    tmix_prefetch_take(&p.pf, &p.pf_bytes);
    { const long long nthr = (long long)grid.x * grid.y * (LW ? LW : WM * WN * KS) * 64, lines = (p.pf_bytes + 127) >> 7;
      p.pf_per = p.pf ? (int)((lines + nthr - 1) / nthr) : 0; }
    kern<<<grid, (WM * WN * KS + LW) * 64, SMEM, st>>>(p);
    TMIX_LAUNCH_CHECK();
    return TMIX_OK;
}


template <int BM, int BN, int WM, int WN, int NS, int CONV, int LW = 0, int PH = 0, int KS = 1, int CSOK = 1>
int launch_cs(Params& p, int batch, hipStream_t st) {
    const bool no_trans = p.n_trans_begin < 0;
    if constexpr (CONV == 1 && (LW == 0 || LW == 2) && PH < 4) {
        if (p.S1) return p.cs_out ? launch_cfg<BM, BN, WM, WN, NS, CONV, LW, PH, KS, 1, 2, 1>(p, batch, st) : launch_cfg<BM, BN, WM, WN, NS, CONV, LW, PH, KS, 0, 2, 1>(p, batch, st);
    }
    if constexpr (CSOK) { if (p.cs_out) return launch_cfg<BM, BN, WM, WN, NS, CONV, LW, PH, KS, 1, 2>(p, batch, st); }
    if constexpr (LW && PH >= 4) { if (p.f8copy) return launch_cfg<BM, BN, WM, WN, NS, CONV, LW, PH, KS, 0, 4>(p, batch, st); }
    if constexpr (!CONV) { if (no_trans && p.epilogue == TMIX_EPI_GEGLU && (p.wide & 2)) return launch_cfg<BM, BN, WM, WN, NS, CONV, LW, PH, KS, 0, 1>(p, batch, st); }
    if (no_trans && p.epilogue != TMIX_EPI_GEGLU && (p.wide & 1)) return launch_cfg<BM, BN, WM, WN, NS, CONV, LW, PH, KS, 0, 2>(p, batch, st);
    if constexpr (!CONV) { if (!no_trans && p.epilogue != TMIX_EPI_GEGLU && (p.wide & 1) && (p.wide & 4)) return launch_cfg<BM, BN, WM, WN, NS, CONV, LW, PH, KS, 0, 3>(p, batch, st); }
    return launch_cfg<BM, BN, WM, WN, NS, CONV, LW, PH, KS, 0, 0>(p, batch, st);
}

inline int no_kernel(int cfg) { TMIX_FAIL(TMIX_EINVAL, "gemm: no kernel for tile_cfg %d", cfg); }
int launch_group0(int cfg, int conv, int f8, Params& p, int batch, hipStream_t st);
int launch_group1(int cfg, int conv, int f8, Params& p, int batch, hipStream_t st);
int launch_group2(int cfg, int conv, int f8, Params& p, int batch, hipStream_t st);
int launch_group3(int cfg, int conv, int f8, Params& p, int batch, hipStream_t st);
int launch_group4(int cfg, int conv, int f8, Params& p, int batch, hipStream_t st);
int launch_group5(int cfg, int conv, int f8, Params& p, int batch, hipStream_t st);
bool w22_eligible(const Params& p, int conv, int f8);
int launch_w22(Params& p, int batch, hipStream_t st, int l2_prefetcher = 0);
bool ff1p_eligible(const Params& p, int conv, int f8, int batch);
int launch_ff1p(Params& p, hipStream_t st);
bool convh_eligible(const Params& p, int conv, int f8);
int launch_convh(Params& p, hipStream_t st);
struct QAExtra { const void* K; int64_t ldk, strideK; const void* Vt; int64_t ldvt, strideVt; void* O; int64_t ldo; int rows_per_image, Skv; float scale; };
int launch_qattn(Params& p, const QAExtra& x, int batch, hipStream_t st);
// ... 3 lines not shown
```

tweediemix_amd/i2vgen.py:

```python
from __future__ import annotations

import ctypes as C
import os
from dataclasses import dataclass

import torch

from . import lib as L
from . import ops
from .unet import UNetPlan, BF16, F32, refine_group, run_chains, SHARED as U_SHARED
from .weights import fold_layernorm, interleave_geglu


@dataclass
class I2VConfig:
    in_channels: int = 4
    out_channels: int = 4
    block_out_channels: tuple = (320, 640, 1280, 1280)
    attn_levels: tuple = (True, True, True, False)
    layers_per_block: int = 2
    norm_groups: int = 32
    cross_dim: int = 1024
    head_dim: int = 64
    transformer_in_heads: int = 8
    ctx_pool: int = 32

    @property
    def time_embed_dim(self):
        return self.block_out_channels[0] * 4


FULL = I2VConfig()
TINY = I2VConfig(block_out_channels=(64, 128, 128, 128), cross_dim=128, transformer_in_heads=2, ctx_pool=8)


def _sites(cfg):
    ch, nb = cfg.block_out_channels, len(cfg.block_out_channels)
    t2d, tt = [], [("transformer_in", ch[0], cfg.transformer_in_heads * cfg.head_dim)]
    for bi, co in enumerate(ch):
        for j in range(cfg.layers_per_block):
            if cfg.attn_levels[bi]:
                t2d.append((f"down_blocks.{bi}.attentions.{j}", co)); tt.append((f"down_blocks.{bi}.temp_attentions.{j}", co, co))
    t2d.append(("mid_block.attentions.0", ch[-1])); tt.append(("mid_block.temp_attentions.0", ch[-1], ch[-1]))
    for ui in range(nb):
        bi = nb - 1 - ui
        for j in range(cfg.layers_per_block + 1):
            if cfg.attn_levels[bi]:
                t2d.append((f"up_blocks.{ui}.attentions.{j}", ch[bi])); tt.append((f"up_blocks.{ui}.temp_attentions.{j}", ch[bi], ch[bi]))
    return t2d, tt


class I2VWeights:

    def __init__(self, cfg: I2VConfig, sd: dict, device="cuda"):
        self.cfg, self.device = cfg, torch.device(device)
        self.kind, self.K = "none", 0
        dev = self.device
        self.raw = {k: v for k, v in sd.items() if k.startswith(("image_latents_", "context_embedding", "fps_embedding"))}
        t = {}
        g = lambda n: sd[n].to(dev)
        bf = lambda x: x.to(dev, BF16).contiguous()
        f32 = lambda x: x.to(dev, F32).contiguous()
        for name, v in sd.items():
            if name in self.raw or name == "conv_in.weight":
                continue
            if name.endswith(".bias") or v.dim() == 1:
                t[name] = f32(v)
            elif v.dim() == 5:
                t[name] = bf(v.to(dev)[:, :, :, 0, 0].permute(0, 2, 1))
            elif v.dim() == 4 and v.shape[-1] == 3:
                t[name] = bf(v.to(dev).permute(0, 2, 3, 1))
            elif v.dim() == 4:
                t[name] = bf(v.to(dev).reshape(v.shape[0], v.shape[1]))
            elif v.dim() == 2 and ".attn" not in name and ".ff.net.0.proj" not in name:
                t[name] = bf(v)
        t["conv_in.weight"] = f32(g("conv_in.weight").permute(0, 2, 3, 1))

        def fold(key, w, norm, bias=None):
            wp, cs, tt = fold_layernorm(w.to(dev, F32), g(norm + ".weight"), g(norm + ".bias"), bias)
            t[key], t[key + ".colsum"], t[key + ".bias"] = wp, cs, tt

        def ff(tb):
            wp, cs, tt = fold_layernorm(g(tb + ".ff.net.0.proj.weight").to(F32), g(tb + ".norm3.weight"), g(tb + ".norm3.bias"),
                                        g(tb + ".ff.net.0.proj.bias"))
            t[tb + ".ff1"] = interleave_geglu(wp, None)[0].contiguous()
            csi, bi = interleave_geglu(cs[:, None], tt)
            t[tb + ".ff1.colsum"], t[tb + ".ff1.bias"] = csi[:, 0].contiguous(), bi.contiguous()

        t2d, tt = _sites(cfg)
        for pfx, _c in t2d:
            tb = pfx + ".transformer_blocks.0"
            a1, a2 = tb + ".attn1", tb + ".attn2"
            fold(a1 + ".qkv", torch.cat([g(a1 + ".to_q.weight"), g(a1 + ".to_k.weight"), g(a1 + ".to_v.weight")]), tb + ".norm1")
            t[a1 + ".out"] = bf(g(a1 + ".to_out.0.weight"))
            fold(a2 + ".q", g(a2 + ".to_q.weight"), tb + ".norm2")
            t[a2 + ".out"] = bf(g(a2 + ".to_out.0.weight"))
            t[a2 + ".kv_rows"] = bf(torch.cat([g(a2 + ".to_k.weight"), g(a2 + ".to_v.weight")])[None])
            ff(tb)
        for pfx, _c, _inner in tt:
            tb = pfx + ".transformer_blocks.0"
            for a, norm in ((tb + ".attn1", tb + ".norm1"), (tb + ".attn2", tb + ".norm2")):
                fold(a + ".qkv", torch.cat([g(a + ".to_q.weight"), g(a + ".to_k.weight"), g(a + ".to_v.weight")]), norm)
                t[a + ".out"] = bf(g(a + ".to_out.0.weight"))
            ff(tb)
        self.t = t

    def __getitem__(self, k):
        return self.t[k]

    def stacked_time_proj(self):
        if getattr(self, "_tproj", None) is None:
            names = sorted(k[:-len(".time_emb_proj.weight")] for k in self.t if k.endswith(".time_emb_proj.weight"))
            w = torch.cat([self.t[n + ".time_emb_proj.weight"] for n in names], 0).contiguous()
            b = torch.cat([self.t[n + ".time_emb_proj.bias"].float() for n in names], 0).contiguous()
            st = [0]
            for n in names:
                st.append(st[-1] + self.t[n + ".time_emb_proj.weight"].shape[0])
            self._tproj = (w, b, torch.tensor(st, device=w.device, dtype=torch.int32), names)
        return self._tproj

    def conv2_with_shortcut(self, name):
        k = name + ".conv2+shortcut"
        if k + ".weight" not in self.t:
            self.t[k + ".weight"] = ops.shortcut_weight(self.t[name + ".conv2.weight"], self.t[name + ".conv_shortcut.weight"])
            self.t[k + ".bias"] = (self.t[name + ".conv2.bias"] + self.t[name + ".conv_shortcut.bias"]).contiguous()
        return self.t[k + ".weight"], self.t[k + ".bias"]


@torch.no_grad()
def conditioning(W: I2VWeights, fps, image_latents, image_embeddings, encoder_hidden_states):
    cfg, dev = W.cfg, W.device
    p = {k: v.to(dev, F32).contiguous() for k, v in W.raw.items()}
    lin = lambda x, n, **kw: ops.linear_f32(x, p[n + ".weight"], p[n + ".bias"], **kw)
    conv = lambda x, n, **kw: ops.conv3x3_f32(x, p[n + ".weight"], p[n + ".bias"], **kw)
    B, Cc, Fr, H, Wd = image_latents.shape
    il = image_latents.to(dev, F32)
    sin = torch.empty(B, cfg.block_out_channels[0], device=dev, dtype=F32)
    L.check(L.load().tmix_timestep_embedding(fps.to(dev, F32).contiguous().data_ptr(), sin.data_ptr(), B, cfg.block_out_channels[0],
                                             torch.cuda.current_stream().cuda_stream), "tmix_timestep_embedding")
    fps_emb = lin(lin(sin, "fps_embedding.0", act_out=True), "fps_embedding.2")
    n = "image_latents_context_embedding"
    v = conv(il[:, :, 0].contiguous(), n + ".0", silu=True)
    v = ops.adaptive_avgpool_f32(v, cfg.ctx_pool, cfg.ctx_pool)
    v = conv(conv(v, n + ".3", stride=2, silu=True), n + ".5", stride=2)
    ctx_img = v.permute(0, 2, 3, 1).reshape(B, -1, cfg.cross_dim)
    e = lin(lin(image_embeddings.to(dev, F32).contiguous(), "context_embedding.0", act_out=True), "context_embedding.2").view(B, cfg.in_channels, cfg.cross_dim)
    context = torch.cat([encoder_hidden_states.to(dev, F32), ctx_img, e], dim=1)
    n = "image_latents_proj_in"
    x = il.permute(0, 2, 1, 3, 4).reshape(B * Fr, Cc, H, Wd).contiguous()
    x = conv(conv(conv(x, n + ".0", silu=True), n + ".2", silu=True), n + ".4")
    il_feat = ops.i2v_temporal_encoder(x, B, Fr, p, "image_latents_temporal_encoder")
    return fps_emb, context, il_feat


# ... 316 lines not shown
```

tweediemix_amd/lib.py:

```python
from __future__ import annotations

import ctypes as C
import os

_HERE = os.path.dirname(os.path.abspath(__file__))
LIB_PATH = os.path.join(_HERE, "lib", "libtmix_hip.so")
LIB_PATH = os.environ.get("TMIX_LIB", LIB_PATH)

OK, EINVAL, ESHAPE, EARCH, EALIGN = 0, -1, -2, -3, -4
F32, F16, BF16 = 0, 1, 2
STEP_FUSION, STEP_PLAIN, STEP_RESAMPLE = 0, 1, 2
EPI_NONE, EPI_GEGLU, EPI_F32OUT, EPI_GELU, EPI_QUICKGELU = 0, 1, 2, 3, 4
CONV_S1, CONV_S2, CONV_UP2, CONV_T3, CONV_S2A = 0, 1, 2, 3, 4
F8_A_BLOCK_SCALES, F8_GEGLU_OUT, F8_COPY_OUT = 1, 2, 4
TILE_AUTO, TILE_COUNT = 0, 26
TILE_CANDIDATES = (1, 2, 3, 4, 5, 7, 12, 13, 14, 15, 16, 17, 18, 19, 20, 21, 22)
TILE_EXCLUSIVE = (13, 14, 15, 22, 24)
TILE_CONV_HALO = 26

i32, i64, f32, vp = C.c_int32, C.c_int64, C.c_float, C.c_void_p


class GemmDesc(C.Structure):
    _fields_ = [("A", vp), ("lda", i64), ("strideA", i64),
                ("W", vp), ("ldw", i64), ("strideW", i64),
                ("C", vp), ("ldc", i64), ("strideC", i64),
                ("bias", vp), ("strideBias", i64),
                ("residual", vp), ("ldr", i64), ("strideR", i64),
                ("rowgroup_bias", vp), ("rows_per_group", i32),
                ("Ct", vp), ("ldct", i64), ("strideCt", i64),
                ("n_trans_begin", i32),
                ("M", i32), ("N", i32), ("K", i32), ("batch", i32),
                ("epilogue", i32), ("tile_cfg", i32),
                ("row_stats_out", vp), ("strideStatsOut", i64), ("ldStatsOut", i64),
                ("ln_stats", vp), ("strideLnStats", i64), ("ldLnStats", i64),
                ("ln_colsum", vp), ("strideLnColsum", i64), ("ln_inv_c", f32), ("ln_eps", f32),
                ("ln_parts", C.c_int32), ("reserved0", C.c_int32),
                ("col_stats_out", vp), ("w_period", C.c_int32), ("reserved1", C.c_int32)]


class ConvDesc(C.Structure):
    _fields_ = [("X", vp), ("Wt", vp), ("Y", vp), ("bias", vp), ("batch_bias", vp), ("residual", vp),
                ("B", i32), ("H", i32), ("W", i32), ("Cin", i32), ("Cout", i32), ("mode", i32), ("tile_cfg", i32),
                ("batch_bias_images", i32), ("col_stats_out", vp), ("S1", vp), ("S2", vp), ("S1_channels", i32), ("S2_channels", i32)]


SIGNATURES = {
    "tmix_version": (C.c_int, []),
    "tmix_last_error_string": (C.c_char_p, []),
    "tmix_check_device": (C.c_int, []),
    "tmix_env_refresh": (None, []),
    "tmix_prof_begin": (C.c_int, [vp, C.c_int, C.c_int]),
    "tmix_prof_end": (C.c_int, []),
    "tmix_fused_tweedie_step": (C.c_int, [vp, vp, C.c_int, vp, vp, vp, C.c_int, C.c_int, i64, C.c_int,
                                          f32, f32, f32, f32, f32, C.c_int, vp]),
    "tmix_fused_tweedie_step_dev": (C.c_int, [vp, vp, C.c_int, vp, i64, vp, vp, C.c_int, C.c_int, i64, C.c_int, C.c_int,
                                              C.c_int, vp, vp]),
    "tmix_fused_tweedie_step_keep_dev": (C.c_int, [vp, vp, C.c_int, vp, i64, vp, vp, C.c_int, C.c_int, i64, C.c_int, C.c_int,
                                                   C.c_int, vp, vp, i64, vp, i64, vp, i64, vp]),
    "tmix_step_prologue": (C.c_int, [vp, vp, vp, vp, C.c_int, C.c_int, i64, vp]),
    "tmix_gemm_bf16": (C.c_int, [C.POINTER(GemmDesc), vp]),
    "tmix_gemm_prefetch_next": (C.c_int, [vp, i64, vp]),
    "tmix_gemm_fp8": (C.c_int, [C.POINTER(GemmDesc), vp, vp, vp]),
    "tmix_gemm_q_cross_attn": (C.c_int, [C.POINTER(GemmDesc), vp, i64, i64, vp, i64, i64, vp, i64, C.c_int, C.c_int, f32, vp]),
    "tmix_quantize_fp8_rows": (C.c_int, [vp, i64, vp, i64, vp, i64, C.c_int, vp]),
    "tmix_conv3x3_nhwc": (C.c_int, [C.POINTER(ConvDesc), vp]),
    "tmix_conv3x3_nhwc_fp8": (C.c_int, [C.POINTER(ConvDesc), vp, vp, vp]),
    "tmix_conv_in": (C.c_int, [vp, vp, vp, vp, C.c_int, C.c_int, C.c_int, C.c_int, C.c_int, vp]),
    "tmix_conv_in_pre": (C.c_int, [vp, vp, vp, vp, C.c_int, C.c_int, C.c_int, C.c_int, C.c_int, vp, vp, vp]),
    "tmix_softmax_rows": (C.c_int, [vp, i64, vp, i64, i64, C.c_int, f32, vp]),
    "tmix_softmax_rows_causal": (C.c_int, [vp, i64, vp, i64, i64, C.c_int, f32, C.c_int, vp]),
    "tmix_softmax_rows_masked": (C.c_int, [vp, i64, vp, i64, i64, C.c_int, C.c_int, f32, vp]),
    "tmix_affine_clamp": (C.c_int, [vp, vp, i64, f32, f32, f32, f32, vp]),
    "tmix_conv_out": (C.c_int, [vp, vp, vp, vp, C.c_int, C.c_int, C.c_int, C.c_int, C.c_int, vp]),
    "tmix_attn_fwd": (C.c_int, [vp, i64, i64, vp, i64, i64, vp, i64, i64, vp, i64, i64,
                                C.c_int, C.c_int, C.c_int, C.c_int, f32, vp]),
    "tmix_attn_fwd_f8": (C.c_int, [vp, i64, i64, vp, i64, i64, vp, i64, i64, vp, i64, vp, i64,
                                   C.c_int, C.c_int, C.c_int, C.c_int, f32, vp]),
    "tmix_attn_split_ws_bytes": (i64, [C.c_int, C.c_int, C.c_int, C.c_int]),
    "tmix_attn_fwd_ws": (C.c_int, [vp, i64, i64, vp, i64, i64, vp, i64, i64, vp, i64, i64,
                                   C.c_int, C.c_int, C.c_int, C.c_int, f32, vp, i64, vp]),
    "tmix_attn_fwd_f8_ws": (C.c_int, [vp, i64, i64, vp, i64, i64, vp, i64, i64, vp, i64, vp, i64,
                                      C.c_int, C.c_int, C.c_int, C.c_int, f32, vp, i64, vp]),
    "tmix_groupnorm_nhwc_launches": (C.c_int, [i64, C.c_int, C.c_int]),
    "tmix_groupnorm_ws_chunks": (C.c_int, [i64]),
    "tmix_groupnorm_ws_floats": (i64, [C.c_int, C.c_int, C.c_int]),
    "tmix_groupnorm_nhwc": (C.c_int, [vp, C.c_int, vp, C.c_int, vp, vp, vp, vp, C.c_int, i64, C.c_int, f32,
                                      C.c_int, vp]),
    "tmix_groupnorm_nhwc_pre": (C.c_int, [vp, C.c_int, vp, C.c_int, vp, vp, vp, vp, C.c_int, i64, C.c_int, f32,
                                          C.c_int, vp, C.c_int, vp, C.c_int, vp]),
    "tmix_groupnorm_nhwc_pre_f8": (C.c_int, [vp, C.c_int, vp, C.c_int, vp, vp, vp, vp, vp, C.c_int, i64, C.c_int, f32,
                                             C.c_int, vp, C.c_int, vp, C.c_int, vp]),
    "tmix_layernorm": (C.c_int, [vp, vp, vp, vp, i64, C.c_int, f32, vp]),
    "tmix_zero": (C.c_int, [vp, i64, vp]),
    "tmix_temporal_attn": (C.c_int, [vp, i64, vp, i64, C.c_int, C.c_int, i64, C.c_int, f32, vp]),
    "tmix_vpred_step": (C.c_int, [vp, vp, vp, C.c_int, i64, f32, f32, f32, f32, f32, vp]),
# ... 52 lines not shown
```

tweediemix_amd/ops.py:

```python
from __future__ import annotations

import ctypes as C

import numpy as np
import torch

from . import lib as L

BF16 = torch.bfloat16


def _stream() -> int:
    return torch.cuda.current_stream().cuda_stream


def _p(t):
    return None if t is None else t.data_ptr()


def _need_cuda(*ts):
    for t in ts:
        if t is not None and not t.is_cuda:
            raise L.TmixError("tweediemix_amd ops need device tensors (no CPU fallback exists)")


_EPS_DT = {torch.float32: L.F32, torch.float16: L.F16, torch.bfloat16: L.BF16}


def step_coeffs(at, at_next):
    at, an = np.float32(at), np.float32(at_next)
    one = np.float32(1)
    return (float(np.sqrt(at)), float(np.sqrt(one - at)), float(np.sqrt(an)), float(np.sqrt(one - an)))


def fused_tweedie_step(x, eps, masks, mode, K, g, at, at_next, is_last=False, out_x=None, out_x0=None):
    _need_cuda(x, eps, masks)
    lib = L.load()
    assert x.dtype == torch.float32 and x.is_contiguous() and eps.is_contiguous()
    Cc, h, w = x.shape[-3], x.shape[-2], x.shape[-1]
    rows = eps.shape[0]
    need = {L.STEP_FUSION: K + 1, L.STEP_PLAIN: 2, L.STEP_RESAMPLE: K + 1}[mode]
    if rows < need:
        raise L.TmixError(f"tweedie step mode {mode} needs {need} eps rows, got {rows}")
    if mode == L.STEP_FUSION:
        assert masks is not None and masks.dtype == torch.float32 and masks.is_contiguous() and masks.shape[0] == K
        assert masks.numel() == K * h * w
    if out_x is None:
        out_x = torch.empty_like(x)
    sa, s1, san, s1n = step_coeffs(at, at_next)
    L.check(lib.tmix_fused_tweedie_step(_p(x), _p(eps), _EPS_DT[eps.dtype], _p(masks), _p(out_x), _p(out_x0),
                                        K, Cc, h * w, mode, float(g), sa, s1, san, s1n, int(bool(is_last)),
                                        _stream()), "tmix_fused_tweedie_step")
    return out_x


def _seed_stride(t, seeds, extent, what):
    assert t.dtype == torch.float32 and t.is_contiguous() and t.shape[0] in (1, seeds) and t.numel() == t.shape[0] * extent, (what, tuple(t.shape))
    return 0 if t.shape[0] == 1 else extent


def fused_tweedie_step_keep_dev(x, eps, masks, mode, K, params, keep_x0, keep_eps, keep_w, out_x=None, out_x0=None):
    _need_cuda(x, eps, masks, params, keep_x0, keep_eps, keep_w)
    assert x.dtype == torch.float32 and x.is_contiguous() and eps.is_contiguous() and params.dtype == torch.float32 and params.numel() >= 8
    S, Cc, h, w = x.shape
    n, hw = Cc * h * w, h * w
    assert eps.shape[0] % S == 0
    rows = eps.shape[0] // S
    mss = 0
    if mode == L.STEP_FUSION:
        assert masks is not None and masks.dtype == torch.float32 and masks.is_contiguous() and masks.numel() in (K * hw, S * K * hw)
        mss = 0 if masks.numel() == K * hw else K * hw
    if out_x is None:
        out_x = torch.empty_like(x)
    L.check(L.load().tmix_fused_tweedie_step_keep_dev(
        _p(x), _p(eps), _EPS_DT[eps.dtype], _p(masks), mss, _p(out_x), _p(out_x0), K, Cc, hw, mode, rows, S, _p(params),
        _p(keep_x0), _seed_stride(keep_x0, S, n, "keep_x0"), _p(keep_eps), _seed_stride(keep_eps, S, n, "keep_eps"),
        _p(keep_w), _seed_stride(keep_w, S, hw, "keep_w"), _stream()), "tmix_fused_tweedie_step_keep_dev")
    return out_x


def stats_parts(N, tile_cfg):
    n = L.load().tmix_gemm_stats_parts(int(N), int(tile_cfg))
    assert n > 0, (N, tile_cfg)
    return n

# ... 122 lines not shown
    return out if out is not None else kw.get("out_f32")


def q_cross_attn_args(k, vt, out, rows_per_image, scale):
    assert k.dtype == BF16 and vt.dtype == BF16 and out.dtype == BF16 and k.stride(2) == 1 and vt.stride(2) == 1 and out.stride(-1) == 1
    o2 = out.reshape(-1, out.shape[-1])
    assert o2.data_ptr() == out.data_ptr()
    return (k.data_ptr(), k.stride(1), k.stride(0), vt.data_ptr(), vt.stride(1), vt.stride(0), o2.data_ptr(), o2.stride(0),
            int(rows_per_image), int(k.shape[1]), float(scale))


def gemm_q_cross_attn(a, w, k, vt, rows_per_image, scale, out=None, **kw):
    _need_cuda(a, w, k, vt)
    if out is None:
        out = torch.empty(*a.shape[:-1], w.shape[-2], device=a.device, dtype=BF16)
    d = make_gemm_desc(a, w, None, **kw)
    L.check(L.load().tmix_gemm_q_cross_attn(C.byref(d), *q_cross_attn_args(k, vt, out, rows_per_image, scale), _stream()), "tmix_gemm_q_cross_attn")
    return out


def quantize_fp8_rows(x, q=None, scale=None):
    _need_cuda(x)
    assert x.dtype == BF16 and x.stride(-1) == 1
    K = x.shape[-1]
    if K > 8192:
        xf = x.float()
        amax = xf.abs().amax(dim=-1)
        bits = (amax.float() * torch.tensor(1.0 / 448.0, dtype=torch.float32, device=amax.device)).view(torch.int32)
        e = (((bits >> 23) & 0xff) - 127 + ((bits & 0x7fffff) != 0).to(torch.int32)).clamp(-127, 127)
        e = torch.where(amax > 0, e, torch.zeros_like(e)).float()
        qt = (xf * torch.exp2(-e).unsqueeze(-1)).to(torch.float8_e4m3fn).view(torch.uint8)
        st = (e + 127).to(torch.uint8)
        if q is not None:
            q.copy_(qt); qt = q
        if scale is not None:
            scale.copy_(st); st = scale
        return qt.contiguous(), st.contiguous()
    x2 = x.reshape(-1, K)
    if q is None:
        q = torch.empty(x.shape, device=x.device, dtype=torch.uint8)
    if scale is None:
        scale = torch.empty(x.shape[:-1], device=x.device, dtype=torch.uint8)
    q2 = q.view(-1, K)
    L.check(L.load().tmix_quantize_fp8_rows(x2.data_ptr(), x2.stride(0), q2.data_ptr(), q2.stride(0), scale.data_ptr(), x2.shape[0], K,
                                            _stream()), "tmix_quantize_fp8_rows")
    return q, scale


def dequantize_fp8_rows(q, scale):
    return q.view(torch.float8_e4m3fn).float() * torch.exp2(scale.float() - 127.0).unsqueeze(-1)


def gemm_fp8(a8, sa, w8, sw, out=None, a_block_scales=False, f8_out=None, f8_copy=None, **kw):
    _need_cuda(a8, w8, sa, sw)
    lib = L.load()
    if f8_out is not None:
        c8, cs = f8_out
        assert kw.get("geglu") and c8.dtype == torch.uint8 and cs.dtype == torch.uint8 and cs.is_contiguous() and c8.stride(-1) == 1
        d = make_gemm_desc(a8, w8, None, **kw)
        c3 = c8 if c8.dim() == 3 else c8.unsqueeze(0)
        d.C, d.ldc, d.strideC = c3.data_ptr(), c3.stride(1), (c3.stride(0) if c3.shape[0] > 1 else 0)
        d.Ct, d.ldct = cs.data_ptr(), cs.shape[1]
        d.reserved0 = L.F8_GEGLU_OUT | (L.F8_A_BLOCK_SCALES if a_block_scales else 0)
        L.check(lib.tmix_gemm_fp8(C.byref(d), sa.data_ptr(), sw.data_ptr(), _stream()), "tmix_gemm_fp8")
        return c8, cs
    if out is None and kw.get("out_f32") is None:
        N = w8.shape[-2]
        No = N // 2 if kw.get("geglu") else (kw["n_trans_begin"] if kw.get("out_t") is not None else N)
        out = torch.empty(*a8.shape[:-1], No, device=a8.device, dtype=BF16)
    assert sa.dtype == torch.uint8 and sw.dtype == torch.uint8 and sa.is_contiguous() and sw.is_contiguous()
    d = make_gemm_desc(a8, w8, out, **kw)
    if a_block_scales:
        assert sa.dim() == 2 and sa.shape[0] == a8.shape[-1] // 32
        d.reserved0 = L.F8_A_BLOCK_SCALES
    if f8_copy is not None:
        f8_copy.attach(d)
    L.check(lib.tmix_gemm_fp8(C.byref(d), sa.data_ptr(), sw.data_ptr(), _stream()), "tmix_gemm_fp8")
    return out if out is not None else kw.get("out_f32")


def make_conv_desc(x, w, out, bias=None, batch_bias=None, residual=None, mode=L.CONV_S1, tile_cfg=0, bias_images=1, col_stats_out=None,
                   shortcut=None, _fp8=False):
    B, H, W, Cin = x.shape
    Cout = w.shape[0]
    dt = torch.uint8 if _fp8 else BF16
    assert x.dtype == dt and w.dtype == dt and x.is_contiguous() and w.is_contiguous() and out.is_contiguous()
    if shortcut is not None:
        s1, s2 = shortcut
        c1, c2 = s1.shape[-1], (0 if s2 is None else s2.shape[-1])
        assert mode == L.CONV_S1 and tuple(w.shape) == (Cout, 9 * Cin + c1 + c2) and residual is None
        assert s1.dtype == BF16 and s1.is_contiguous() and s1.numel() == B * H * W * c1 and (s2 is None or (s2.dtype == BF16 and s2.is_contiguous() and s2.numel() == B * H * W * c2))
    else:
        assert tuple(w.shape) == ((Cout, 3, Cin) if mode == L.CONV_T3 else (Cout, 3, 3, Cin))
    d = L.ConvDesc()
    d.X, d.Wt, d.Y = x.data_ptr(), w.data_ptr(), out.data_ptr()
    d.bias, d.batch_bias, d.residual = _p(bias), _p(batch_bias), _p(residual)
    d.B, d.H, d.W, d.Cin, d.Cout, d.mode = B, H, W, Cin, Cout, mode
    d.tile_cfg = tile_cfg
    d.batch_bias_images = bias_images
    if col_stats_out is not None:
        cs = col_stats_out
        assert cs.dtype == torch.float32 and cs.is_contiguous() and tuple(cs.shape) == (out.numel() // Cout // COLSTATS_ROWS, 2, Cout)
        d.col_stats_out = cs.data_ptr()
    if shortcut is not None:
        d.S1, d.S1_channels = s1.data_ptr(), c1
        if s2 is not None:
            d.S2, d.S2_channels = s2.data_ptr(), c2
    return d


def shortcut_weight(w_conv, w_sc):
    Cout = w_conv.shape[0]
    return torch.cat([w_conv.reshape(Cout, -1), w_sc.reshape(Cout, -1)], dim=1).contiguous()


def conv_out_hw(H, W, mode):
    return (H // 2, W // 2) if mode in (L.CONV_S2, L.CONV_S2A) else ((2 * H, 2 * W) if mode == L.CONV_UP2 else (H, W))


def conv3x3_fp8(x8, sx, w8, sw, bias=None, batch_bias=None, residual=None, mode=L.CONV_S1, out=None, tile_cfg=12, col_stats_out=None, bias_images=1):
    _need_cuda(x8, w8, sx, sw)
    lib = L.load()
    B, H, W, Cin = x8.shape
    Ho, Wo = conv_out_hw(H, W, mode)
    if out is None:
        out = torch.empty(B, Ho, Wo, w8.shape[0], device=x8.device, dtype=BF16)
    assert x8.dtype == torch.uint8 and w8.dtype == torch.uint8 and sx.dtype == torch.uint8 and sw.dtype == torch.uint8
    assert x8.is_contiguous() and w8.is_contiguous() and sx.is_contiguous() and sw.is_contiguous() and sx.numel() == B * H * W * Cin // 32 and sw.numel() == w8.shape[0]
    d = make_conv_desc(x8, w8, out, bias, batch_bias, residual, mode, tile_cfg, bias_images=bias_images, col_stats_out=col_stats_out, _fp8=True)
    L.check(lib.tmix_conv3x3_nhwc_fp8(C.byref(d), sx.data_ptr(), sw.data_ptr(), _stream()), "tmix_conv3x3_nhwc_fp8")
    return out


def conv3x3(x, w, bias=None, batch_bias=None, residual=None, mode=L.CONV_S1, out=None, tile_cfg=0, col_stats_out=None, shortcut=None):
    _need_cuda(x, w)
    lib = L.load()
    B, H, W, _ = x.shape
    Ho, Wo = conv_out_hw(H, W, mode)
    if out is None:
        out = torch.empty(B, Ho, Wo, w.shape[0], device=x.device, dtype=BF16)
    d = make_conv_desc(x, w, out, bias, batch_bias, residual, mode, tile_cfg, col_stats_out=col_stats_out, shortcut=shortcut)
    L.check(lib.tmix_conv3x3_nhwc(C.byref(d), _stream()), "tmix_conv3x3_nhwc")
    return out


def conv_in(x_nchw, w_ohwi, bias, out=None):
    _need_cuda(x_nchw, w_ohwi)
    lib = L.load()
    B, Cin, H, W = x_nchw.shape
    Cout = w_ohwi.shape[0]
    assert x_nchw.dtype == torch.float32 and w_ohwi.dtype == torch.float32 and x_nchw.is_contiguous() and w_ohwi.is_contiguous()
    if out is None:
        out = torch.empty(B, H, W, Cout, device=x_nchw.device, dtype=BF16)
    L.check(lib.tmix_conv_in(_p(x_nchw), _p(w_ohwi), _p(bias), _p(out), B, Cin, H, W, Cout, _stream()), "tmix_conv_in")
    return out


def conv_out(x_nhwc, w_ohwi, bias, out=None):
    _need_cuda(x_nhwc, w_ohwi)
    lib = L.load()
    B, H, W, Cin = x_nhwc.shape
    Cout = w_ohwi.shape[0]
    assert x_nhwc.dtype == BF16 and w_ohwi.dtype == BF16 and x_nhwc.is_contiguous() and w_ohwi.is_contiguous()
    if out is None:
        out = torch.empty(B, Cout, H, W, device=x_nhwc.device, dtype=torch.float32)
    L.check(lib.tmix_conv_out(_p(x_nhwc), _p(w_ohwi), _p(bias), _p(out), B, Cin, H, W, Cout, _stream()), "tmix_conv_out")
    return out


def attention_split_ws(B, H, Sq, Skv, device):
    n = L.load().tmix_attn_split_ws_bytes(B, H, Sq, Skv)
    return torch.zeros(n, device=device, dtype=torch.uint8) if n > 0 else None


def attention(q, k, vt, H, Skv, scale, out=None, f8_out=None, ws=None):
    _need_cuda(q, k, vt)
    lib = L.load()
    B, Sq = q.shape[0], q.shape[1]
    assert q.dtype == BF16 and k.dtype == BF16 and vt.dtype == BF16
    assert q.stride(2) == 1 and k.stride(2) == 1 and vt.stride(2) == 1
    wsa = (ws.data_ptr(), ws.numel()) if ws is not None else (None, 0)
    if f8_out is not None:
        assert f8_out.rows == B * Sq and f8_out.N == H * 64
        L.check(lib.tmix_attn_fwd_f8_ws(_p(q), q.stride(1), q.stride(0), _p(k), k.stride(1), k.stride(0), _p(vt), vt.stride(1), vt.stride(0),
                                        f8_out.q.data_ptr(), f8_out.N, f8_out.scales.data_ptr(), f8_out.rows,
                                        B, H, Sq, Skv, float(scale), *wsa, _stream()), "tmix_attn_fwd_f8_ws")
        return f8_out
    if out is None:
        out = torch.empty(B, Sq, H * 64, device=q.device, dtype=BF16)
    L.check(lib.tmix_attn_fwd_ws(_p(q), q.stride(1), q.stride(0), _p(k), k.stride(1), k.stride(0),
                                 _p(vt), vt.stride(1), vt.stride(0), _p(out), out.stride(1), out.stride(0),
                                 B, H, Sq, Skv, float(scale), *wsa, _stream()), "tmix_attn_fwd_ws")
    return out


def token_array(tokens):
    tokens = [int(t) for t in tokens]
    return (C.c_int32 * max(1, len(tokens)))(*tokens)


def xattn_token_maps(q, k, tokens, H, Lk=None, rows=(0, 1, None), scale=None, out=None, accumulate=False):
    _need_cuda(q, k)
    assert q.dtype == BF16 and k.dtype == BF16 and q.stride(2) == 1 and k.stride(2) == 1
    B, Sq = q.shape[0], q.shape[1]
    Lk = k.shape[1] if Lk is None else Lk
    row0, step, n = rows
    n = len(range(row0, B, step)) if n is None else n
    if out is None:
        out = torch.zeros(n, len(tokens), Sq, device=q.device, dtype=torch.float32)
    assert out.dtype == torch.float32 and out.is_contiguous() and tuple(out.shape) == (n, len(tokens), Sq)
    scale = 64 ** -0.5 if scale is None else scale
    L.check(L.load().tmix_xattn_token_maps(_p(q), q.stride(1), q.stride(0), _p(k), k.stride(1), k.stride(0), _p(out), B, H, Sq, Lk,
                                           row0, step, n, token_array(tokens), len(tokens), int(bool(accumulate)), float(scale),
                                           _stream()), "tmix_xattn_token_maps")
    return out


def groupnorm_ws(B, C, groups, device):
    return torch.empty(L.load().tmix_groupnorm_ws_floats(B, C, groups), device=device, dtype=torch.float32)


def groupnorm(x1, gamma, beta, groups=32, eps=1e-5, silu=False, x2=None, out=None, ws=None, colstats=None, f8_out=None):
    _need_cuda(x1, gamma, beta)
# ... 242 lines not shown
```

tweediemix_amd/unet.py:

```python
from __future__ import annotations

import ctypes as C
import json
import os
from dataclasses import dataclass

import torch

from . import lib as L
from . import ops
from .weights import fold_layernorm, interleave_geglu

BF16 = torch.bfloat16
F32 = torch.float32


@dataclass
class UNetConfig:
    in_channels: int = 4
    out_channels: int = 4
    block_out_channels: tuple = (320, 640, 1280)
    layers_per_block: int = 2
    transformer_layers: tuple = (0, 2, 10)
    head_dim: int = 64
# ... 9 lines not shown
    @property
    def add_in_dim(self):
        return self.pooled_dim + 6 * self.addition_time_embed_dim


    @classmethod
    def from_diffusers(cls, cfg: dict):
        ch = tuple(cfg["block_out_channels"])
        tl = cfg.get("transformer_layers_per_block", 1)
        tl = tuple(tl) if isinstance(tl, (list, tuple)) else (tl,) * len(ch)
        down = cfg.get("down_block_types", ["CrossAttnDownBlock2D"] * len(ch))
        tl = tuple(n if "CrossAttn" in t else 0 for n, t in zip(tl, down))
        heads = cfg.get("attention_head_dim", 8)
        heads = tuple(heads) if isinstance(heads, (list, tuple)) else (heads,) * len(ch)
        hd = {c // h for c, h, n in zip(ch, heads, tl) if n}
        if hd != {64}:
            raise ValueError(f"attention head size {sorted(hd)}: the attention kernel is built for 64 (SDXL)")
        add = cfg.get("addition_time_embed_dim", 256)
        return cls(in_channels=cfg.get("in_channels", 4), out_channels=cfg.get("out_channels", 4), block_out_channels=ch,
                   layers_per_block=cfg.get("layers_per_block", 2), transformer_layers=tl, head_dim=64,
                   cross_dim=cfg.get("cross_attention_dim", 2048),
                   pooled_dim=cfg.get("projection_class_embeddings_input_dim", 2816) - 6 * add,
                   addition_time_embed_dim=add, norm_groups=cfg.get("norm_num_groups", 32))


SDXL = UNetConfig()
TINY = UNetConfig(block_out_channels=(64, 128, 256), transformer_layers=(0, 1, 2), cross_dim=128,
                  pooled_dim=64, addition_time_embed_dim=32)


def transformer_sites(cfg: UNetConfig):
    out = []
    ch = cfg.block_out_channels
    nb = len(ch)
    for bi in range(nb):
        for j in range(cfg.layers_per_block):
            if cfg.transformer_layers[bi]:
                out.append((f"down_blocks.{bi}.attentions.{j}", ch[bi], cfg.transformer_layers[bi]))
    out.append(("mid_block.attentions.0", ch[-1], cfg.transformer_layers[-1]))
    for ui in range(nb):
        bi = nb - 1 - ui
        for j in range(cfg.layers_per_block + 1):
            if cfg.transformer_layers[bi]:
                out.append((f"up_blocks.{ui}.attentions.{j}", ch[bi], cfg.transformer_layers[bi]))
    return out


def attention_blocks(cfg: UNetConfig):
    return [(f"{p}.transformer_blocks.{i}", c) for p, c, n in transformer_sites(cfg) for i in range(n)]


class UNetWeights:

    def __init__(self, cfg: UNetConfig, sd: dict, device="cuda", concepts=None, lora_mode="merged"):
        self.cfg, self.device = cfg, torch.device(device)
        self.kind = concepts[0] if concepts else "none"
        self.K = len(concepts[1]) if concepts else 0
        assert lora_mode in ("merged", "lowrank")
        self.lora_mode = lora_mode if self.kind == "lora" else "merged"
        self._fp8 = {}
        self._tproj = None
        dev = self.device
        t = {}

        def g(name):
            return sd[name].to(dev)

        def bf(x):
            return x.to(dev, BF16).contiguous()

        def f32(x):
            return x.to(dev, F32).contiguous()

        for name, v in sd.items():
            if name.endswith(".bias") or ".norm" in name and name.endswith(".weight") or name.startswith("conv_norm_out"):
                t[name] = f32(v)
        t["conv_in.weight"] = f32(g("conv_in.weight").permute(0, 2, 3, 1))
        t["conv_out.weight"] = bf(g("conv_out.weight").permute(0, 2, 3, 1))
        for name, v in sd.items():
            if not name.endswith(".weight") or name in ("conv_in.weight", "conv_out.weight"):
                continue
            if v.dim() == 4 and v.shape[-1] == 3:
                t[name] = bf(v.to(dev).permute(0, 2, 3, 1))
            elif v.dim() == 4:
                t[name] = bf(v.to(dev).reshape(v.shape[0], v.shape[1]))
            elif v.dim() == 2 and ".attn" not in name and ".ff.net.0.proj" not in name:
                t[name] = bf(v)
        lora = concepts[1] if self.kind == "lora" else None
        custom = concepts[1] if self.kind == "custom" else None

        def merged(base, key, which):
            rows = [base.to(dev, F32)]
            for csd in lora:
                kd, ku = f"{key}.processor.to_{which}_lora.down.weight", f"{key}.processor.to_{which}_lora.up.weight"
                if kd in csd and ku in csd:
                    rows.append(rows[0] + csd[ku].to(dev, F32) @ csd[kd].to(dev, F32))
                else:
                    rows.append(rows[0])
            return torch.stack(rows)

        def lowrank(key, base, a, whiches, norm=None):
            nw, nsets = len(whiches), 1 + len(lora)
            P = 4 * nw
            assert nsets * P <= 64, "low-rank LoRA: (1 + concepts) x 4 x fused projections must fit the 64 pad columns"
            N, Kin = base.shape
            n1 = N // nw
            U = torch.zeros(N, 64, device=dev, dtype=F32)
            Dm = torch.zeros(nsets * P, Kin, device=dev, dtype=F32)
            for si, csd in enumerate(lora):
                for c, which in enumerate(whiches):
                    kd, ku = f"{a}.processor.to_{which}_lora.down.weight", f"{a}.processor.to_{which}_lora.up.weight"
                    if kd in csd and ku in csd:
                        col = ((si + 1) * nw + c) * 4
                        U[c * n1:(c + 1) * n1, col:col + 4] = csd[ku].to(dev, F32)
                        Dm[(si + 1) * P + c * 4:(si + 1) * P + c * 4 + 4] = csd[kd].to(dev, F32)
            t[key + ".lr"] = torch.cat([base.to(dev, BF16), U.to(BF16)], dim=1).contiguous()
            if norm is not None:
                gm, bt = g(norm + ".weight").to(F32), g(norm + ".bias").to(F32)
                Dp = (Dm * gm).to(BF16)
                t[key + ".lr.D"], t[key + ".lr.dcolsum"], t[key + ".lr.dbias"] = Dp.contiguous(), Dp.float().sum(1).contiguous(), (Dm @ bt).contiguous()
            else:
                t[key + ".lr.D"] = Dm.to(BF16).contiguous()
            t[key + ".lr.P"] = P

        def fold(key, w, norm, bias=None):
            wp, cs, tt = fold_layernorm(w.to(dev, F32), g(norm + ".weight"), g(norm + ".bias"), bias)
            t[key], t[key + ".colsum"], t[key + ".bias"] = wp, cs, tt

        for tb, _c in attention_blocks(cfg):
            a1, a2 = tb + ".attn1", tb + ".attn2"
            n1, n2, n3 = tb + ".norm1", tb + ".norm2", tb + ".norm3"
            fold(a1 + ".qkv", torch.cat([g(a1 + ".to_q.weight"), g(a1 + ".to_k.weight"), g(a1 + ".to_v.weight")]), n1)
            t[a1 + ".out"] = bf(g(a1 + ".to_out.0.weight"))
            fold(a2 + ".q", g(a2 + ".to_q.weight"), n2)
            t[a2 + ".out"] = bf(g(a2 + ".to_out.0.weight"))
            kv_rows = [torch.cat([g(a2 + ".to_k.weight"), g(a2 + ".to_v.weight")]).to(F32)]
            if custom is not None:
                for csd in custom:
                    ck = csd[a2 + ".to_k.weight"].to(dev, F32) if a2 + ".to_k.weight" in csd else kv_rows[0][:kv_rows[0].shape[0] // 2]
                    cv = csd[a2 + ".to_v.weight"].to(dev, F32) if a2 + ".to_v.weight" in csd else kv_rows[0][kv_rows[0].shape[0] // 2:]
                    kv_rows.append(torch.cat([ck, cv]))
            if lora is not None:
                mk = merged(g(a2 + ".to_k.weight"), a2, "k")
                mv = merged(g(a2 + ".to_v.weight"), a2, "v")
                kv_rows = [torch.cat([mk[i], mv[i]]) for i in range(mk.shape[0])]
                if self.lora_mode == "lowrank":
                    lowrank(a1 + ".qkv", t[a1 + ".qkv"], a1, ("q", "k", "v"), n1)
                    lowrank(a1 + ".out", t[a1 + ".out"], a1, ("out",))
                    lowrank(a2 + ".q", t[a2 + ".q"], a2, ("q",), n2)
                    lowrank(a2 + ".out", t[a2 + ".out"], a2, ("out",))
                else:
                    fold(a1 + ".qkv_rows", torch.cat([merged(g(a1 + ".to_q.weight"), a1, "q"),
                                                      merged(g(a1 + ".to_k.weight"), a1, "k"),
                                                      merged(g(a1 + ".to_v.weight"), a1, "v")], dim=1), n1)
                    t[a1 + ".out_rows"] = bf(merged(g(a1 + ".to_out.0.weight"), a1, "out"))
                    fold(a2 + ".q_rows", merged(g(a2 + ".to_q.weight"), a2, "q"), n2)
                    t[a2 + ".out_rows"] = bf(merged(g(a2 + ".to_out.0.weight"), a2, "out"))
            t[a2 + ".kv_rows"] = bf(torch.stack(kv_rows))
            wp, cs, tt = fold_layernorm(g(tb + ".ff.net.0.proj.weight").to(F32), g(n3 + ".weight"), g(n3 + ".bias"),
                                        g(tb + ".ff.net.0.proj.bias"))
            t[tb + ".ff1"] = interleave_geglu(wp, None)[0].contiguous()
            csi, bi = interleave_geglu(cs[:, None], tt)
            t[tb + ".ff1.colsum"], t[tb + ".ff1.bias"] = csi[:, 0].contiguous(), bi.contiguous()
        self.t = t

    def __getitem__(self, k):
# ... 358 lines not shown
        elif kw.get("ln_stats") is not None:
            self._ln_links[-1][1].append(d)
        self.keep.append(d)
        self._hint_weights(w)
        self._emit(self.lib.tmix_gemm_bf16, C.byref(d))
        fl = 2 * d.M * d.N * d.K * d.batch
        self.flops += fl
        self.gemm_flops += fl
        self.launches["gemm"].append((d, fl))
        self._tunable.append((len(self.ops) - 1, "gemm", d))
        self.op_meta[len(self.ops) - 1] = ("gemm", fl, d)
        return out

    def _gemm_fp8(self, a, key, out, f8_out=None, f8_copy=None, **kw):
        name, rows = key if isinstance(key, tuple) else (key, None)
        w8, sw = self.W.fp8(name, rows)
        flags = 0
        if isinstance(a, tuple):
            a8, sa = a
            flags |= L.F8_A_BLOCK_SCALES
            owned = ()
        else:
            K = a.shape[-1]
            a8 = self.arena.get(*a.shape, dtype=torch.uint8)
            sa = self.arena.get(*a.shape[:-1], dtype=torch.uint8)
            a2 = a.reshape(-1, K)
            assert a2.data_ptr() == a.data_ptr() and a2.stride(1) == 1
            self._emit(self.lib.tmix_quantize_fp8_rows, a2.data_ptr(), a2.stride(0), a8.data_ptr(), K, sa.data_ptr(), a2.shape[0], K)
            owned = (a8, sa)
        Ng, Kg = w8.shape[-2], w8.shape[-1]
        rows_g = a8.shape[-2] * (a8.shape[0] if a8.dim() == 3 else 1)
        lock = self.fp8_tile and f8_out is None and kw.get("out_t") is None and Kg % 128 == 0 and Ng % 160 == 0 and Ng <= 1280
        many = not (Kg >= 2560 or rows_g * Ng <= 4096 * 1280)
        if lock and (not many or kw.get("row_stats_out") is not None):
            kw.setdefault("tile_cfg", self.fp8_tile)
        if kw.get("row_stats_out") is not None:
            kw.setdefault("tile_cfg", 17)
        d = ops.make_gemm_desc(a8, w8, None if f8_out is not None else out, **kw)
        if f8_out is not None:
            c8, cs = f8_out
            assert kw.get("geglu") and c8.dim() == 2 and c8.stride(1) == 1 and cs.is_contiguous()
            d.C, d.ldc, d.strideC = c8.data_ptr(), c8.stride(0), 0
            d.Ct, d.ldct = cs.data_ptr(), cs.shape[1]
            flags |= L.F8_GEGLU_OUT
        d.reserved0 = flags
        if f8_copy is not None:
            f8_copy.attach(d)
            self.keep.append(f8_copy)
        if kw.get("row_stats_out") is not None:
            self._ln_links.append((d, []))
        elif kw.get("ln_stats") is not None:
            self._ln_links[-1][1].append(d)
        self.keep += [d, a8, sa]
        self._hint_weights(w8)
        self._emit(self.lib.tmix_gemm_fp8, C.byref(d), sa.data_ptr(), sw.data_ptr())
        fl = 2 * d.M * d.N * d.K * d.batch
        self.flops += fl
        self.gemm_flops += fl
        self.launches["gemm"].append((d, fl))
        self.op_meta[len(self.ops) - 1] = ("gemm_fp8", fl, d)
        if owned:
            self.arena.put(*owned)
        return out

    def _conv(self, x, wname, Hh, Ww, Cin, Cout, mode=L.CONV_S1, batch_bias=None, residual=None, bias_images=1, shortcut=None):
        Ho, Wo = ops.conv_out_hw(Hh, Ww, mode)
        out = self.arena.get(self.B, Ho * Wo, Cout)
        if isinstance(x, tuple):
            assert shortcut is None
            x8, sx = x
            w8, sw = self.W.fp8(wname + ".weight")
            d = ops.make_conv_desc(x8.view(self.B, Hh, Ww, Cin), w8.view(Cout, 3, 3, Cin), out.view(self.B, Ho, Wo, Cout), self.W[wname + ".bias"], batch_bias,
                                   residual, mode, tile_cfg=self.fp8_conv_tile, bias_images=bias_images,
                                   col_stats_out=self._colstats(out, self.B * Ho * Wo, Ho * Wo, Cout), _fp8=True)
            self.keep += [d, x8, sx, w8, sw]
            self._hint_weights(w8)
            self._emit(self.lib.tmix_conv3x3_nhwc_fp8, C.byref(d), sx.data_ptr(), sw.data_ptr())
            fl = 2 * self.B * Ho * Wo * Cout * 9 * Cin
            self.flops += fl
            self.launches["conv"].append((d, fl))
            self.op_meta[len(self.ops) - 1] = ("conv_fp8", fl, d)
            return out
        w, bias, sc, csc = self.W[wname + ".weight"], self.W[wname + ".bias"], None, 0
        if shortcut is not None:
            w, bias = self.W.conv2_with_shortcut(shortcut[0])
            sc = (shortcut[1], shortcut[2])
            csc = w.shape[1] - 9 * Cin
        d = ops.make_conv_desc(x.view(self.B, Hh, Ww, Cin), w, out.view(self.B, Ho, Wo, Cout),
                               bias, batch_bias, residual, mode, bias_images=bias_images,
                               col_stats_out=self._colstats(out, self.B * Ho * Wo, Ho * Wo, Cout),
                               shortcut=sc)
        self.keep.append(d)
        self._hint_weights(w)
        self._emit(self.lib.tmix_conv3x3_nhwc, C.byref(d))
        fl = 2 * self.B * Ho * Wo * Cout * (9 * Cin + csc)
        self.flops += fl
        self.launches["conv"].append((d, fl))
        self._tunable.append((len(self.ops) - 1, "conv", d))
        self.op_meta[len(self.ops) - 1] = ("conv", fl, d)
        return out

    def _ln_stats(self, S, Cc):
        pm = (Cc + 127) // 128
        return self._ln_buf[:pm * self.B * S * 2].view(pm, self.B * S, 2)

    def _link_ln(self):
        for _i, kind, d in self._tunable:
            if kind == "gemm" and (d.reserved0 & L.F8_COPY_OUT):
                d.tile_cfg = ops.f8copy_tile(d.tile_cfg)
        for prod, cons in self._ln_links:
            parts = ops.stats_parts(prod.N, prod.tile_cfg)
            for c in cons:
                c.ln_parts = parts

    def _q_attn(self, h, key, k, vt, ao, S, Cc, ln):
        W = self.W
        shp = (self.B, S) if self.routed else (self.B * S,)
        kw = {"ln_stats": ln, "ln_colsum": self._rows(key, ".colsum") if self.routed else W[key + ".colsum"],
              "bias": self._rows(key, ".bias") if self.routed else W[key + ".bias"]}
        w = self._rows(key) if self.routed else W[key]
        d = ops.make_gemm_desc(h.view(*shp, Cc), w, None, **kw)
        self._ln_links[-1][1].append(d)
        args = ops.q_cross_attn_args(k, vt, ao, S, self.cfg.head_dim ** -0.5)
        self.keep += [d, k, vt, ao]
        self._hint_weights(w)
        self._emit(self.lib.tmix_gemm_q_cross_attn, C.byref(d), *args)
        fl = 2 * d.M * d.N * d.K * d.batch
        fla = 4 * self.B * (Cc // 64) * S * k.shape[1] * 64
        self.flops += fl + fla
        self.gemm_flops += fl
        self.launches["gemm"].append((d, fl))
        self.op_meta[len(self.ops) - 1] = ("gemm", fl + fla, d)
        return ao

    def _attn(self, q, k, vt, out, H, Sq, Skv, f8_out=None):
        ws = None
        if os.environ.get("TMIX_ATTN_SPLIT"):
            wkey = (self.B, H, Sq, Skv)
            if wkey not in self._attn_ws:
                self._attn_ws[wkey] = ops.attention_split_ws(*wkey, q.device)
            ws = self._attn_ws[wkey]
        wsa = (ws.data_ptr(), ws.numel()) if ws is not None else (None, 0)
        if f8_out is not None:
            args = (q.data_ptr(), q.stride(1), q.stride(0), k.data_ptr(), k.stride(1), k.stride(0),
                    vt.data_ptr(), vt.stride(1), vt.stride(0), f8_out.q.data_ptr(), f8_out.N, f8_out.scales.data_ptr(), f8_out.rows,
                    self.B, H, Sq, Skv, self.cfg.head_dim ** -0.5, *wsa)
            self._emit(self.lib.tmix_attn_fwd_f8_ws, *args)
            self.keep.append(f8_out)
        else:
            args = (q.data_ptr(), q.stride(1), q.stride(0), k.data_ptr(), k.stride(1), k.stride(0),
                    vt.data_ptr(), vt.stride(1), vt.stride(0), out.data_ptr(), out.stride(1), out.stride(0),
                    self.B, H, Sq, Skv, self.cfg.head_dim ** -0.5, *wsa)
            self._emit(self.lib.tmix_attn_fwd_ws, *args)
        fl = 4 * self.B * H * Sq * Skv * 64
        self.flops += fl
        self.launches["attn"].append((args, fl))
        self.op_meta[len(self.ops) - 1] = ("attn", fl, ("attn", self.B, H, Sq, Skv))
        return out

    def _probe_level(self, Hh):
        if not self.token_maps:
            return None
        lvl = (self.h // Hh).bit_length() - 1
        return lvl if lvl in self.token_maps else None

    def _token_maps(self, q, a2, H, S, lvl):
        sp, k, m = self.token_spec, self.kv.k[a2], self.token_maps[lvl]
        assert m.shape[2] == S
        self._emit(self.lib.tmix_xattn_token_maps, q.data_ptr(), q.stride(1), q.stride(0), k.data_ptr(), k.stride(1), k.stride(0),
                   m.data_ptr(), self.B, H, S, self.kv.Lk, sp.row0, sp.row_step, sp.n_rows, self._tok_arr, m.shape[1], 1,
                   self.cfg.head_dim ** -0.5)

    def _vt_buf(self, Cc, S):
        ld = (S + 7) // 8 * 8
        key = (Cc, ld)
        if key not in self._vt:
            self._vt[key] = torch.zeros(self.B, Cc, ld, device=self.dev, dtype=BF16)
        return self._vt[key]
# ... 265 lines not shown
        A.put(x)
        self._emit(lib.tmix_conv_out, y.data_ptr(), W["conv_out.weight"].data_ptr(), W["conv_out.bias"].data_ptr(),
                   self.eps.data_ptr(), B, C0, Hh, Ww, cfg.out_channels)
        self.flops += 2 * B * Hh * Ww * 9 * (cfg.in_channels * C0 + C0 * cfg.out_channels)
        self.ops = [(fn, tuple(a)) for fn, a in self.ops]

    def issued_meta(self):
        return [self.op_meta[i] for i in range(len(self.ops)) if i in self.op_meta]

    def run(self, stream=None):
        st = stream if stream is not None else torch.cuda.current_stream().cuda_stream
        for fn, args in self.ops:
            rc = fn(*args, st)
            if rc:
                L.check(rc, fn.__name__)

    def __call__(self, latent, t):
        self.latent.copy_(latent)
        self.t_dev.fill_(float(t))
        self.run()
        return self.eps

    def norm_condition(self, latent, t):
        self.latent.copy_(latent)
        self.t_dev.fill_(float(t))
        st = torch.cuda.current_stream().cuda_stream
        prods = {id(d) for d, _c in self._ln_links}
        out = []
        for i, (fn, args) in enumerate(self.ops):
            rc = fn(*args, st)
            if rc:
                L.check(rc, fn.__name__)
            m = self.op_meta.get(i)
            if not m or m[0] not in ("gemm", "gemm_fp8") or id(m[2]) not in prods:
                continue
            d = m[2]
            torch.cuda.synchronize()
            parts = ops.stats_parts(d.N, d.tile_cfg)
            base = (d.row_stats_out - self._ln_buf.data_ptr()) // 4
            rows = torch.arange(d.M, device=self.dev)
            s = torch.zeros(d.batch, d.M, 2, device=self.dev, dtype=torch.float64)
            for bz in range(d.batch):
                for q in range(parts):
                    off = base + bz * d.strideStatsOut + (q * d.ldStatsOut + rows) * 2
                    s[bz, :, 0] += self._ln_buf[off].double()
                    s[bz, :, 1] += self._ln_buf[off + 1].double()
            mean = s[..., 0] / d.N
            var = (s[..., 1] / d.N - mean * mean).clamp_min(1e-30)
            r = (mean.abs() / var.sqrt()).flatten()
            out.append((i, d.M * d.batch, d.N, r.max().item(), r.median().item()))
        torch.cuda.synchronize()
        return out


LN_COND_WARN = 16.0


def refine_group(self, top=14, reps=9, verbose=False, cands=None, only_kind=None):
    def timed():
        self.run()
        torch.cuda.synchronize()
        g = torch.cuda.CUDAGraph()
        with torch.cuda.graph(g):
            self.run()
        for _ in range(2):
            g.replay()
        import time as _time
        ts = []
        burst = 3
        for _ in range(reps):
            torch.cuda.synchronize()
            t0 = _time.perf_counter()
            for _b in range(burst):
                g.replay()
            torch.cuda.synchronize()
            ts.append(1e3 * (_time.perf_counter() - t0) / burst)
        return sorted(ts)[len(ts) // 2]

    plans = _plans_of(self)
    weight, members = {}, {}
    for p in plans:
        for _i, kind, d in p._tunable:
            k = p._tune_key(kind, d)
            fl = 2.0 * d.M * d.N * d.K * d.batch if kind == "gemm" else 2.0 * d.B * d.H * d.W * d.Cout * (9 * d.Cin + d.S1_channels + d.S2_channels)
            weight[k] = weight.get(k, 0.0) + fl
            members.setdefault(k, []).append((p, kind, d))
    base = timed()
    if only_kind is not None:
        weight = {k: v for k, v in weight.items() if members[k][0][1] == only_kind}
    for k in sorted(weight, key=weight.get, reverse=True)[:top]:
        cur = members[k][0][2].tile_cfg
        best, best_t = cur, base
        for cfg in (cands or L.TILE_CANDIDATES):
            _p0, kind0, d0 = members[k][0]
            if cfg == cur or (cfg in L.TILE_EXCLUSIVE and len(plans) > 1):
                continue
            if kind0 == "conv" and ops.conv_runs_as(d0, cfg) != cfg:
                continue
            if cfg == L.TILE_CONV_HALO and (kind0 != "conv" or d0.S1_channels):
                continue
            for p, _kind, d in members[k]:
                d.tile_cfg = cfg
            for p in plans:
                p._link_ln()
            if os.environ.get("TMIX_REFINE_TRACE"):
                print(f"    try {k} cfg {cfg}", flush=True)
            t = timed()
            if t < best_t - 0.02:
                best, best_t = cfg, t
        for p, _kind, d in members[k]:
            d.tile_cfg = best
        for p in plans:
            p._link_ln()
        if verbose:
            print(f"  refine {k}: {cur} -> {best}  ({base:.3f} -> {best_t:.3f} ms)", flush=True)
        _TUNE_CACHE[members[k][0][0].tune_ctx + k] = best
        base = best_t
    return base



def _plans_of(plan):
    return list(plan.plans) if hasattr(plan, "plans") else [plan]


def used_tilings(plan):
    out = {}
    for p in _plans_of(plan):
        for _i, kind, d in p._tunable:
            k = f"{kind}:{d.tile_cfg}"
            out[k] = out.get(k, 0) + 1
    return dict(sorted(out.items()))


def tilings_follow_table(plan):
    bad = []
    with open(_TUNE_FILE) as f:
        table = {k: int(v) for k, v in json.load(f).items()}

    def shipped(ctx, key):
        c = table.get(ctx + key)
        if c is None and ctx:
            c = table.get(key)
            if ctx == SHARED and c in L.TILE_EXCLUSIVE:
                c = None
        return c

    for p in _plans_of(plan):
        for _i, kind, d in p._tunable:
            k = p._tune_key(kind, d)
            want = shipped(p.tune_ctx, k)
            if kind == "gemm" and (d.reserved0 & L.F8_COPY_OUT) and want is not None:
                want = ops.f8copy_tile(want)
            if want != d.tile_cfg:
                bad.append((k, d.tile_cfg, want))
    return not bad, bad


UNetPlan.refine = lambda self, **kw: refine_group(self, **kw)


class PlanGroup:

    def __init__(self, W: UNetWeights, h: int, w: int, ehs: torch.Tensor, wsel, pooled: torch.Tensor,
                 time_ids: torch.Tensor, routed: bool, n_groups: int, fp8: bool = False):
        B = ehs.shape[0]
        assert B % n_groups == 0
# ... 49 lines not shown
```

tweediemix_amd/vae.py:

```python
from __future__ import annotations

import ctypes as C

import torch

from . import lib as L
from . import ops
from .unet import _Arena

BF16, F32 = torch.bfloat16, torch.float32

FULL = dict(block_out_channels=(128, 256, 512, 512), layers_per_block=2, latent_channels=4, out_channels=3, groups=32)
TINY = dict(block_out_channels=(64, 64, 128, 128), layers_per_block=1, latent_channels=4, out_channels=3, groups=32)


def param_shapes(cfg) -> dict:
    P = {}
    ch = list(reversed(cfg["block_out_channels"]))
    lc = cfg["latent_channels"]

    def conv(n, i, o, k=3):
        P[n + ".weight"] = (o, i, k, k)
        P[n + ".bias"] = (o,)

# ... 21 lines not shown
            ci = co
        if i < len(ch) - 1:
            conv(f"decoder.up_blocks.{i}.upsamplers.0.conv", co, co)
    vec2("decoder.conv_norm_out", ch[-1])
    conv("decoder.conv_out", ch[-1], cfg["out_channels"])
    return P


def encoder_param_shapes(cfg) -> dict:
    P = {}
    ch = list(cfg["block_out_channels"])
    lc = cfg["latent_channels"]

    def conv(n, i, o, k=3):
        P[n + ".weight"] = (o, i, k, k)
        P[n + ".bias"] = (o,)

    def vec2(n, c):
        P[n + ".weight"] = (c,)
        P[n + ".bias"] = (c,)

    def resnet(n, ci, co):
        vec2(n + ".norm1", ci); conv(n + ".conv1", ci, co); vec2(n + ".norm2", co); conv(n + ".conv2", co, co)
        if ci != co:
            conv(n + ".conv_shortcut", ci, co, 1)

    conv("encoder.conv_in", cfg["out_channels"], ch[0])
    ci = ch[0]
    for i, co in enumerate(ch):
        for j in range(cfg["layers_per_block"]):
            resnet(f"encoder.down_blocks.{i}.resnets.{j}", ci, co)
            ci = co
        if i < len(ch) - 1:
            conv(f"encoder.down_blocks.{i}.downsamplers.0.conv", co, co)
    resnet("encoder.mid_block.resnets.0", ci, ci)
    vec2("encoder.mid_block.attentions.0.group_norm", ci)
    for nm in ("to_q", "to_k", "to_v", "to_out.0"):
        P[f"encoder.mid_block.attentions.0.{nm}.weight"] = (ci, ci)
        P[f"encoder.mid_block.attentions.0.{nm}.bias"] = (ci,)
    resnet("encoder.mid_block.resnets.1", ci, ci)
    vec2("encoder.conv_norm_out", ci)
    conv("encoder.conv_out", ci, 2 * lc)
    conv("quant_conv", 2 * lc, 2 * lc, 1)
    return P


def synthetic_state_dict(cfg, seed=4321, device="cpu", nontrivial=False, encoder=False):
    gen = torch.Generator(device=device).manual_seed(seed)
    sd = {}
    for name, shape in (encoder_param_shapes(cfg) if encoder else param_shapes(cfg)).items():
        is_norm = "norm" in name
        if name.endswith(".bias"):
            v = torch.randn(shape, generator=gen, device=device) * 0.05 if nontrivial else torch.zeros(shape, device=device)
        elif is_norm:
            v = torch.ones(shape, device=device) + (0.1 * torch.randn(shape, generator=gen, device=device) if nontrivial else 0)
        else:
            fan = 1
            for s_ in shape[1:]:
                fan *= s_
            v = torch.randn(shape, generator=gen, device=device) * fan ** -0.5
            if ".conv2." in name or ".to_out.0." in name:
                v = v * 0.3
        sd[name] = v.to(BF16).float() if not name.startswith(("post_quant_conv", "decoder.conv_in", "quant_conv", "encoder.conv_in")) else v.float()
    return sd


class VAEDecoderPlan:

    def __init__(self, cfg, sd, B, h, w, inv_scale, device="cuda"):
        self.cfg, self.B, self.h, self.w = cfg, B, h, w
        self.dev = torch.device(device)
        self.lib = L.load()
        self.ops, self.keep = [], []
        self.arena = _Arena(self.dev)
        self.flops = 0
        dev = self.dev
        t = {}
        for k, v in sd.items():
            v = v.to(dev)
            if k.endswith(".bias") or "norm" in k:
                t[k] = v.to(F32).contiguous()
            elif v.dim() == 4 and v.shape[-1] == 3 and not k.startswith("decoder.conv_in"):
                t[k] = v.permute(0, 2, 3, 1).to(BF16).contiguous()
            elif v.dim() == 4 and v.shape[-1] == 1 and not k.startswith("post_quant"):
                t[k] = v.reshape(v.shape[0], v.shape[1]).to(BF16).contiguous()
            elif v.dim() == 2:
                t[k] = v.to(BF16).contiguous()
        t["decoder.conv_in.weight"] = sd["decoder.conv_in.weight"].to(dev, F32).permute(0, 2, 3, 1).contiguous()
        a = "decoder.mid_block.attentions.0"
        t[a + ".qkv"] = torch.cat([t[a + ".to_q.weight"], t[a + ".to_k.weight"], t[a + ".to_v.weight"]]).contiguous()
        t[a + ".qkv.bias"] = torch.cat([t[a + ".to_q.bias"], t[a + ".to_k.bias"], t[a + ".to_v.bias"]]).contiguous()
        self.t = t
        pq = sd["post_quant_conv.weight"].float().reshape(4, 4) * float(inv_scale)
        self._pre_w = (C.c_float * 16)(*[float(x) for x in pq.reshape(-1)])
        self._pre_b = (C.c_float * 4)(*[float(x) for x in sd["post_quant_conv.bias"].float()])
        self.latent = torch.zeros(B, 4, h, w, device=dev, dtype=F32)
        self.image = torch.zeros(B, cfg["out_channels"], 8 * h, 8 * w, device=dev, dtype=F32)
        self._gn_ws = ops.groupnorm_ws(B, 4096, cfg["groups"], dev)
        self._build()

    def _emit(self, fn, *a):
        self.ops.append((fn, a))

    def _gn(self, x, Cc, HW, name, silu):
        out = self.arena.get(self.B, HW, Cc)
        self._emit(self.lib.tmix_groupnorm_nhwc, x.data_ptr(), Cc, None, 0, out.data_ptr(), self.t[name + ".weight"].data_ptr(),
                   self.t[name + ".bias"].data_ptr(), self._gn_ws.data_ptr(), self.B, HW, self.cfg["groups"], 1e-6, int(silu))
        return out

    def _conv(self, x, name, Hh, Ww, Ci, Co, mode=L.CONV_S1, residual=None):
        Ho, Wo = ops.conv_out_hw(Hh, Ww, mode)
        out = self.arena.get(self.B, Ho * Wo, Co)
        d = ops.make_conv_desc(x.view(self.B, Hh, Ww, Ci), self.t[name + ".weight"], out.view(self.B, Ho, Wo, Co),
                               self.t[name + ".bias"], None, residual, mode)
        self.keep.append(d)
        self._emit(self.lib.tmix_conv3x3_nhwc, C.byref(d))
        self.flops += 2 * self.B * Ho * Wo * Co * 9 * Ci
        return out

    def _gemm(self, a, w, out, **kw):
        d = ops.make_gemm_desc(a, w, out, **kw)
        self.keep.append(d)
        self._emit(self.lib.tmix_gemm_bf16, C.byref(d))
        self.flops += 2 * d.M * d.N * d.K * d.batch
        return d

    def _resnet(self, x, Ci, Co, Hh, Ww, name):
        A, B = self.arena, self.B
        HW = Hh * Ww
        h1 = self._gn(x, Ci, HW, name + ".norm1", True)
        h2 = self._conv(h1, name + ".conv1", Hh, Ww, Ci, Co)
        A.put(h1)
        h3 = self._gn(h2, Co, HW, name + ".norm2", True)
        A.put(h2)
        if Ci != Co:
            sc = A.get(B, HW, Co)
            self._gemm(x.view(B * HW, Ci), self.t[name + ".conv_shortcut.weight"], sc.view(B * HW, Co), bias=self.t[name + ".conv_shortcut.bias"])
        else:
            sc = x
        out = self._conv(h3, name + ".conv2", Hh, Ww, Co, Co, residual=sc)
        A.put(h3)
        if Ci != Co:
            A.put(sc)
        return out

    def _attn(self, x, Cc, Hh, Ww, name):
        A, B, t = self.arena, self.B, self.t
        S = Hh * Ww
        g = self._gn(x, Cc, S, name + ".group_norm", False)
        qk = A.get(B, S, 2 * Cc)
        vt = torch.zeros(B, Cc, S, device=self.dev, dtype=BF16)
        self.keep.append(vt)
        self._gemm(g.view(B, S, Cc), t[name + ".qkv"], qk, bias=t[name + ".qkv.bias"], out_t=vt, n_trans_begin=2 * Cc)
        A.put(g)
        scores = torch.empty(B, S, S, device=self.dev, dtype=F32)
        probs = torch.empty(B, S, S, device=self.dev, dtype=BF16)
        self.keep += [scores, probs]
        d = ops.make_gemm_desc(qk[:, :, :Cc], qk[:, :, Cc:], None)
        d.C, d.ldc, d.strideC, d.epilogue = scores.data_ptr(), S, S * S, L.EPI_F32OUT
        self.keep.append(d)
        self._emit(self.lib.tmix_gemm_bf16, C.byref(d))
        self.flops += 2 * B * S * S * Cc
        self._emit(self.lib.tmix_softmax_rows, scores.data_ptr(), S, probs.data_ptr(), S, B * S, S, Cc ** -0.5)
        ao = A.get(B, S, Cc)
        self._gemm(probs, vt, ao)
        A.put(qk)
        out = A.get(B, S, Cc)
        self._gemm(ao.view(B * S, Cc), t[name + ".to_out.0.weight"], out.view(B * S, Cc), bias=t[name + ".to_out.0.bias"],
                   residual=x.view(B * S, Cc))
        A.put(ao)
        return out

    def _build(self):
        cfg, A, B, lib, t = self.cfg, self.arena, self.B, self.lib, self.t
        ch = list(reversed(cfg["block_out_channels"]))
        Hh, Ww = self.h, self.w
        x = A.get(B, Hh * Ww, ch[0])
        self._emit(lib.tmix_conv_in_pre, self.latent.data_ptr(), t["decoder.conv_in.weight"].data_ptr(),
                   t["decoder.conv_in.bias"].data_ptr(), x.data_ptr(), B, 4, Hh, Ww, ch[0], self._pre_w, self._pre_b)
        x2 = self._resnet(x, ch[0], ch[0], Hh, Ww, "decoder.mid_block.resnets.0"); A.put(x)
        x3 = self._attn(x2, ch[0], Hh, Ww, "decoder.mid_block.attentions.0"); A.put(x2)
        x = self._resnet(x3, ch[0], ch[0], Hh, Ww, "decoder.mid_block.resnets.1"); A.put(x3)
        ci = ch[0]
        for i, co in enumerate(ch):
            for j in range(cfg["layers_per_block"] + 1):
                x2 = self._resnet(x, ci, co, Hh, Ww, f"decoder.up_blocks.{i}.resnets.{j}")
                A.put(x)
                x, ci = x2, co
            if i < len(ch) - 1:
                x2 = self._conv(x, f"decoder.up_blocks.{i}.upsamplers.0.conv", Hh, Ww, co, co, mode=L.CONV_UP2)
                A.put(x)
                x = x2
                Hh, Ww = Hh * 2, Ww * 2
        y = self._gn(x, ch[-1], Hh * Ww, "decoder.conv_norm_out", True)
        A.put(x)
        raw = torch.empty_like(self.image)
        self.keep.append(raw)
        self._emit(lib.tmix_conv_out, y.data_ptr(), t["decoder.conv_out.weight"].data_ptr(), t["decoder.conv_out.bias"].data_ptr(),
                   raw.data_ptr(), B, ch[-1], Hh, Ww, cfg["out_channels"])
        self._emit(lib.tmix_affine_clamp, raw.data_ptr(), self.image.data_ptr(), raw.numel(), 0.5, 0.5, 0.0, 1.0)
# ... 102 lines not shown
```

Before: 33.11.

## Fold nearest-upsample into four-phase 2x2 convolutions for upsampler convs

Adds a folded upsampling conv mode that turns nearest-2x upsample followed by a 3x3 conv into four per-phase 2x2 convolutions on the low-resolution input. Weights are pre-summed per phase at load time, and the kernel picks the phase weight slice per tile and scatters output rows to their interleaved positions. This cuts the reduction length from 9*Cin to 4*Cin, removing more than half the upsampler conv FLOPs in the UNet and VAE. In exchange it adds strided, non-contiguous output stores, extra index math, a tiling constraint (H*W must be a multiple of the tile rows), and bf16 rounding of the summed weights.

```diff
diff --git a/include/tmix.h b/include/tmix.h
--- a/include/tmix.h
+++ b/include/tmix.h
@@ -100,7 +100,7 @@
 int tmix_gemm_tile_shape(int tile_cfg, int* bm, int* bn);
 int tmix_gemm_stats_parts(int N, int tile_cfg);
 
-enum { TMIX_CONV_S1 = 0, TMIX_CONV_S2 = 1, TMIX_CONV_UP2 = 2, TMIX_CONV_T3 = 3, TMIX_CONV_S2A = 4 };
+enum { TMIX_CONV_S1 = 0, TMIX_CONV_S2 = 1, TMIX_CONV_UP2 = 2, TMIX_CONV_T3 = 3, TMIX_CONV_S2A = 4, TMIX_CONV_UP2F = 5 };
 typedef struct {
     const void* X;
     const void* Wt;
diff --git a/tweediemix_amd/csrc/gemm_conv.hip b/tweediemix_amd/csrc/gemm_conv.hip
--- a/tweediemix_amd/csrc/gemm_conv.hip
+++ b/tweediemix_amd/csrc/gemm_conv.hip
@@ -250,16 +250,21 @@
     if (d->B <= 0 || d->H <= 0 || d->W <= 0 || d->Cin <= 0 || d->Cout <= 0) TMIX_FAIL(TMIX_ESHAPE, "conv3x3: empty problem");
     if (d->Cin % BK) TMIX_FAIL(TMIX_ESHAPE, "conv3x3: Cin=%d must be a multiple of %d", d->Cin, BK);
     if (d->Cout % 4) TMIX_FAIL(TMIX_ESHAPE, "conv3x3: Cout=%d must be a multiple of 4", d->Cout);
-    if (d->mode < TMIX_CONV_S1 || d->mode > TMIX_CONV_S2A) TMIX_FAIL(TMIX_EINVAL, "conv3x3: bad mode %d", d->mode);
+    if (d->mode < TMIX_CONV_S1 || d->mode > TMIX_CONV_UP2F) TMIX_FAIL(TMIX_EINVAL, "conv3x3: bad mode %d", d->mode);
+    const bool fold = d->mode == TMIX_CONV_UP2F;
+    if (fold && (fp8 || d->residual || d->S1 || d->S2)) TMIX_FAIL(TMIX_EINVAL, "conv3x3: the folded upsampling mode takes bf16 operands, no residual and no shortcut taps");
+    if (fold && (d->W < 2 || (int64_t)d->H * d->W * d->W >= (1ll << 32))) TMIX_FAIL(TMIX_ESHAPE, "conv3x3: the folded upsampling mode needs W >= 2 and H * W * W < 2^32");
     if ((d->mode == TMIX_CONV_S2 || d->mode == TMIX_CONV_S2A) && ((d->H | d->W) & 1)) TMIX_FAIL(TMIX_ESHAPE, "conv3x3: stride-2 needs even H,W");
     if (!aligned16(d->X) || !aligned16(d->Wt) || (((uintptr_t)d->Y) & 7)) TMIX_FAIL(TMIX_EALIGN, "conv3x3: pointer alignment");
     if ((d->bias && (((uintptr_t)d->bias) & 15)) || (d->batch_bias && (((uintptr_t)d->batch_bias) & 15))) TMIX_FAIL(TMIX_EALIGN, "conv3x3: bias alignment");
     p = {};
     p.H = d->H; p.Wd = d->W; p.Cin = d->Cin; p.mode = d->mode;
-    p.ntaps = d->mode == TMIX_CONV_T3 ? 3 : 9;
+    p.ntaps = d->mode == TMIX_CONV_T3 ? 3 : (fold ? 4 : 9);
+    if (fold) { p.up_hw = d->H * d->W; p.up_magic = (unsigned)((1ull << 32) / (unsigned)d->W) + 1u; }
     const bool half = d->mode == TMIX_CONV_S2 || d->mode == TMIX_CONV_S2A;
-    p.Ho = half ? d->H / 2 : (d->mode == TMIX_CONV_UP2 ? d->H * 2 : d->H);
-    p.Wo = half ? d->W / 2 : (d->mode == TMIX_CONV_UP2 ? d->W * 2 : d->W);
+    const bool up = d->mode == TMIX_CONV_UP2 || fold;
+    p.Ho = half ? d->H / 2 : (up ? d->H * 2 : d->H);
+    p.Wo = half ? d->W / 2 : (up ? d->W * 2 : d->W);
     const int64_t M = (int64_t)d->B * p.Ho * p.Wo;
     if (M > 0x7fffffff / 4) TMIX_FAIL(TMIX_ESHAPE, "conv3x3: too many output pixels");
     if ((int64_t)d->B * d->H * d->W * d->Cin >= (1ll << 30) || (int64_t)d->Cout * 9 * d->Cin >= (1ll << 30)) TMIX_FAIL(TMIX_ESHAPE, "conv3x3: operand larger than 2 GiB");
@@ -295,17 +300,29 @@
     return TMIX_OK;
 }
 
+static int conv_resolve(const Params& p, int tile_cfg, int& cfg) {
+    const TileChoice r = resolve_tile(traits_of(1, p, 1), tile_cfg);
+    if (r.err) return r.err;
+    if (p.mode == TMIX_CONV_UP2F && (p.up_hw % TILINGS[r.cfg].bm))
+        TMIX_FAIL(TMIX_ESHAPE, "conv3x3: the folded upsampling mode needs H * W = %d to be a multiple of the %d rows of tiling %d (use TMIX_CONV_UP2)", p.up_hw, TILINGS[r.cfg].bm, r.cfg);
+    cfg = r.cfg;
+    return TMIX_OK;
+}
+
 static int conv_entry(const tmix_conv_desc* d, const uint8_t* scale_x, const uint8_t* scale_w, void* stream) {
     Params p;
     if (const int rc = conv_params(d, scale_x, scale_w, p)) return rc;
+    int cfg;
+    if (const int rc = conv_resolve(p, d->tile_cfg, cfg)) return rc;
     return launch(1, p, 1, d->tile_cfg, (hipStream_t)stream);
 }
 
 extern "C" int tmix_conv_resolve_tile(const tmix_conv_desc* d, int fp8_operands) {
     Params p;
     if (const int rc = conv_params(d, fp8_operands ? NO_SCALES : nullptr, fp8_operands ? NO_SCALES : nullptr, p)) return rc;
-    const TileChoice r = resolve_tile(traits_of(1, p, 1), d->tile_cfg);
-    return r.err ? r.err : r.cfg;
+    int cfg;
+    if (const int rc = conv_resolve(p, d->tile_cfg, cfg)) return rc;
+    return cfg;
 }
 
 extern "C" int tmix_conv3x3_nhwc(const tmix_conv_desc* d, void* stream) { return conv_entry(d, nullptr, nullptr, stream); }
diff --git a/tweediemix_amd/csrc/gemm_kernel.h b/tweediemix_amd/csrc/gemm_kernel.h
--- a/tweediemix_amd/csrc/gemm_kernel.h
+++ b/tweediemix_amd/csrc/gemm_kernel.h
@@ -51,6 +51,7 @@
     const float* ln_stats; int64_t strideLnStats, ldLnStats; const float* ln_colsum; int64_t strideLnColsum;
     float ln_inv_c, ln_eps; int ln_parts;
     int H, Wd, Cin, Ho, Wo, mode, ntaps;
+    int up_hw; unsigned up_magic;
     unsigned long long* prof; int prof_detail;
     int wide;
     const unsigned char* scaleA; const unsigned char* scaleW; int64_t strideScaleA, strideScaleW;
@@ -87,6 +88,8 @@
     constexpr bool F8L = PH >= 4;
     constexpr int SCP = (F8L && F8B) ? 1 : 0;
     constexpr int EB = F8 ? 1 : 2;
+    constexpr bool UPF = CONV && !SC && !F8;
+    const bool upf = UPF && p.mode == TMIX_CONV_UP2F;
     constexpr int NW = WM * WN;
     constexpr int TM = BM / WM, TN = BN / WN;
     constexpr int FM = TM / 32, FN = TN / 32;
@@ -151,6 +154,13 @@
 
     const bf16_t* Ab = (const bf16_t*)((const char*)p.A + (int64_t)bz * p.strideA * EB);
     const bf16_t* Wb = (const bf16_t*)((const char*)p.W + (int64_t)bzw * p.strideW * EB);
+    int up_q = 0;
+    if constexpr (CONV) {
+        if (upf) {
+            up_q = __builtin_amdgcn_readfirstlane(m0 / p.up_hw);
+            Wb += (int64_t)(up_q & 3) * p.N * p.ldw;
+        }
+    }
     const __amdgpu_buffer_rsrc_t rsA = __builtin_amdgcn_make_buffer_rsrc((void*)Ab, 0, p.bytesA, 0x00020000);
     const __amdgpu_buffer_rsrc_t rsW = __builtin_amdgcn_make_buffer_rsrc((void*)Wb, 0, p.bytesW, 0x00020000);
 
@@ -168,7 +178,12 @@
             const int b = m / hw, rem = m - b * hw;
             const int py = rem / p.Wo, px = rem - py * p.Wo;
             int iy0, ix0; unsigned par = 0;
-            if (p.mode == TMIX_CONV_S1 || p.mode == TMIX_CONV_T3) { iy0 = py - 1; ix0 = px - 1; }
+            if (upf) {
+                const int ph = rem / p.up_hw, l = rem - ph * p.up_hw;
+                const int sy = l / p.Wd, sx = l - sy * p.Wd;
+                iy0 = sy - 1 + (ph >> 1); ix0 = sx - 1 + (ph & 1);
+            }
+            else if (p.mode == TMIX_CONV_S1 || p.mode == TMIX_CONV_T3) { iy0 = py - 1; ix0 = px - 1; }
             else if (p.mode == TMIX_CONV_S2) { iy0 = 2 * py - 1; ix0 = 2 * px - 1; }
             else if (p.mode == TMIX_CONV_S2A) { iy0 = 2 * py; ix0 = 2 * px; }
             else { iy0 = (py - 1) >> 1; ix0 = (px - 1) >> 1; par = (unsigned)((py - 1) & 1) << 16 | (unsigned)((px - 1) & 1) << 17; }
@@ -176,7 +191,8 @@
 #pragma unroll
             for (int t = 0; t < 9; ++t) {
                 if (t >= p.ntaps) break;
-                const int ky = p.mode == TMIX_CONV_T3 ? t : t / 3, kx = p.mode == TMIX_CONV_T3 ? 1 : t - (t / 3) * 3;
+                const int ky = p.mode == TMIX_CONV_T3 ? t : (upf ? t >> 1 : t / 3);
+                const int kx = p.mode == TMIX_CONV_T3 ? 1 : (upf ? t & 1 : t - (t / 3) * 3);
                 bool ok;
                 if (p.mode == TMIX_CONV_UP2) { const int uy = py + ky - 1, ux = px + kx - 1; ok = (uy >= 0) & (uy < 2 * p.H) & (ux >= 0) & (ux < 2 * p.Wd); }
                 else { const int iy = iy0 + ky, ix = ix0 + kx; ok = (iy >= 0) & (iy < p.H) & (ix >= 0) & (ix < p.Wd); }
@@ -284,7 +300,8 @@
                 return;
             }
         }
-        const int ky = p.mode == TMIX_CONV_T3 ? tap : tap / 3, kx = p.mode == TMIX_CONV_T3 ? 1 : tap - ky * 3;
+        const int ky = p.mode == TMIX_CONV_T3 ? tap : (upf ? tap >> 1 : tap / 3);
+        const int kx = p.mode == TMIX_CONV_T3 ? 1 : (upf ? tap & 1 : tap - ky * 3);
         const unsigned pixb = (unsigned)p.Cin * (unsigned)EB, rowb = (unsigned)p.Wd * pixb;
         if (p.mode == TMIX_CONV_UP2) {
             const unsigned sd = (ky == 2 ? rowb : 0u) + (kx == 2 ? pixb : 0u), ay = ky == 1 ? rowb : 0u, ax = kx == 1 ? pixb : 0u;
@@ -932,6 +949,19 @@
     }
 
     bf16_t* Cb = p.C + (int64_t)bz * p.strideC;
+    int up_mb = 0, up_ob = 0;
+    if constexpr (CONV) {
+        if (upf) { up_mb = up_q * p.up_hw; up_ob = ((up_q >> 2) * p.Ho + ((up_q >> 1) & 1)) * p.Wo + (up_q & 1); }
+    }
+    auto conv_store_row = [&](int m) __attribute__((always_inline)) -> int {
+        if constexpr (CONV) {
+            if (upf) {
+                const unsigned l = (unsigned)(m - up_mb), sy = __umulhi(l, p.up_magic), sx = l - sy * (unsigned)p.Wd;
+                return up_ob + (int)(2u * sy * (unsigned)p.Wo + 2u * sx);
+            }
+        }
+        return m;
+    };
     if (EK == 1 || (EK == 0 && p.epilogue == TMIX_EPI_GEGLU)) {
         if (EK == 1 || (p.wide & 2)) {
             char* stg = smem + w * STG_MAX;
@@ -1110,7 +1140,7 @@
                         uint4 v;
                         v.x = pack_bf2(o[0], o[1]); v.y = pack_bf2(o[2], o[3]); v.z = pack_bf2(o[4], o[5]); v.w = pack_bf2(o[6], o[7]);
                         const bool ok = m < p.M && ncok;
-                        if (ok) *(uint4*)(Cb + (int64_t)m * p.ldc + nc) = v;
+                        if (ok) *(uint4*)(Cb + (int64_t)conv_store_row(m) * p.ldc + nc) = v;
                         if constexpr (F8C && (FL & 4) != 0) {
                             const unsigned u8[4] = {v.x, v.y, v.z, v.w};
                             float f[8], am = 0.f;
@@ -1211,7 +1241,7 @@
                         uint4 v;
                         v.x = pack_bf2(o[0], o[1]); v.y = pack_bf2(o[2], o[3]); v.z = pack_bf2(o[4], o[5]); v.w = pack_bf2(o[6], o[7]);
                         if constexpr (ABL & 32) asm volatile("" :: "v"(v.x), "v"(v.y), "v"(v.z), "v"(v.w));
-                        else *(uint4*)(Cb + (int64_t)m * p.ldc + nc) = v;
+                        else *(uint4*)(Cb + (int64_t)conv_store_row(m) * p.ldc + nc) = v;
                         if constexpr (F8C) if (p.f8copy) {
                             const unsigned u8[4] = {v.x, v.y, v.z, v.w};
                             float f[8], am = 0.f;
@@ -1332,7 +1362,7 @@
                     *(float4*)((float*)p.C + (int64_t)bz * p.strideC + (int64_t)m * p.ldc + n) = make_float4(o[0], o[1], o[2], o[3]);
                 } else {
                     uint2 v; v.x = pack_bf2(o[0], o[1]); v.y = pack_bf2(o[2], o[3]);
-                    *(uint2*)(Cb + (int64_t)m * p.ldc + n) = v;
+                    *(uint2*)(Cb + (int64_t)conv_store_row(m) * p.ldc + n) = v;
                     if (sto) {
                         const float r0 = __uint_as_float(v.x << 16), r1 = __uint_as_float(v.x & 0xffff0000u);
                         const float r2 = __uint_as_float(v.y << 16), r3 = __uint_as_float(v.y & 0xffff0000u);
diff --git a/tweediemix_amd/i2vgen.py b/tweediemix_amd/i2vgen.py
--- a/tweediemix_amd/i2vgen.py
+++ b/tweediemix_amd/i2vgen.py
@@ -70,6 +70,8 @@
                 t[name] = bf(v.to(dev)[:, :, :, 0, 0].permute(0, 2, 1))
             elif v.dim() == 4 and v.shape[-1] == 3:
                 t[name] = bf(v.to(dev).permute(0, 2, 3, 1))
+                if ".upsamplers." in name:
+                    t[name + ".up2f"] = ops.fold_up2_weight(v.to(dev).permute(0, 2, 3, 1))
             elif v.dim() == 4:
                 t[name] = bf(v.to(dev).reshape(v.shape[0], v.shape[1]))
             elif v.dim() == 2 and ".attn" not in name and ".ff.net.0.proj" not in name:
diff --git a/tweediemix_amd/lib.py b/tweediemix_amd/lib.py
--- a/tweediemix_amd/lib.py
+++ b/tweediemix_amd/lib.py
@@ -11,7 +11,7 @@
 F32, F16, BF16 = 0, 1, 2
 STEP_FUSION, STEP_PLAIN, STEP_RESAMPLE = 0, 1, 2
 EPI_NONE, EPI_GEGLU, EPI_F32OUT, EPI_GELU, EPI_QUICKGELU = 0, 1, 2, 3, 4
-CONV_S1, CONV_S2, CONV_UP2, CONV_T3, CONV_S2A = 0, 1, 2, 3, 4
+CONV_S1, CONV_S2, CONV_UP2, CONV_T3, CONV_S2A, CONV_UP2F = 0, 1, 2, 3, 4, 5
 F8_A_BLOCK_SCALES, F8_GEGLU_OUT, F8_COPY_OUT = 1, 2, 4
 TILE_AUTO, TILE_COUNT = 0, 26
 TILE_CANDIDATES = (1, 2, 3, 4, 5, 7, 12, 13, 14, 15, 16, 17, 18, 19, 20, 21, 22)
diff --git a/tweediemix_amd/ops.py b/tweediemix_amd/ops.py
--- a/tweediemix_amd/ops.py
+++ b/tweediemix_amd/ops.py
@@ -1,6 +1,7 @@
 from __future__ import annotations
 
 import ctypes as C
+import os
 
 import numpy as np
 import torch
@@ -289,7 +290,7 @@
 def make_conv_desc(x, w, out, bias=None, batch_bias=None, residual=None, mode=L.CONV_S1, tile_cfg=0, bias_images=1, col_stats_out=None,
                    shortcut=None, _fp8=False):
     B, H, W, Cin = x.shape
-    Cout = w.shape[0]
+    Cout = w.shape[1] if mode == L.CONV_UP2F else w.shape[0]
     dt = torch.uint8 if _fp8 else BF16
     assert x.dtype == dt and w.dtype == dt and x.is_contiguous() and w.is_contiguous() and out.is_contiguous()
     if shortcut is not None:
@@ -298,7 +299,7 @@
         assert mode == L.CONV_S1 and tuple(w.shape) == (Cout, 9 * Cin + c1 + c2) and residual is None
         assert s1.dtype == BF16 and s1.is_contiguous() and s1.numel() == B * H * W * c1 and (s2 is None or (s2.dtype == BF16 and s2.is_contiguous() and s2.numel() == B * H * W * c2))
     else:
-        assert tuple(w.shape) == ((Cout, 3, Cin) if mode == L.CONV_T3 else (Cout, 3, 3, Cin))
+        assert tuple(w.shape) == ((Cout, 3, Cin) if mode == L.CONV_T3 else (4, Cout, 2, 2, Cin) if mode == L.CONV_UP2F else (Cout, 3, 3, Cin))
     d = L.ConvDesc()
     d.X, d.Wt, d.Y = x.data_ptr(), w.data_ptr(), out.data_ptr()
     d.bias, d.batch_bias, d.residual = _p(bias), _p(batch_bias), _p(residual)
@@ -322,7 +323,27 @@
 
 
 def conv_out_hw(H, W, mode):
-    return (H // 2, W // 2) if mode in (L.CONV_S2, L.CONV_S2A) else ((2 * H, 2 * W) if mode == L.CONV_UP2 else (H, W))
+    return (H // 2, W // 2) if mode in (L.CONV_S2, L.CONV_S2A) else ((2 * H, 2 * W) if mode in (L.CONV_UP2, L.CONV_UP2F) else (H, W))
+
+
+def fold_up2_weight(w_ohwi, dtype=BF16):
+    assert w_ohwi.dim() == 4 and tuple(w_ohwi.shape[1:3]) == (3, 3)
+    w = w_ohwi.to(torch.float64 if w_ohwi.dtype == torch.float64 else torch.float32)
+    phases = []
+    for fy in (0, 1):
+        wy = torch.stack([w[:, 0], w[:, 1] + w[:, 2]] if fy == 0 else [w[:, 0] + w[:, 1], w[:, 2]], dim=1)
+        for fx in (0, 1):
+            phases.append(torch.stack([wy[:, :, 0], wy[:, :, 1] + wy[:, :, 2]] if fx == 0 else [wy[:, :, 0] + wy[:, :, 1], wy[:, :, 2]], dim=2))
+    out = torch.stack(phases)
+    return (out if dtype is None else out.to(dtype)).contiguous()
+
+
+def up2_fold_enabled():
+    return os.environ.get("TMIX_UP2_FOLD", "1") != "0"
+
+
+def up2_fold_ok(H, W):
+    return up2_fold_enabled() and W >= 2 and (H * W) % 256 == 0
 
 
 def conv3x3_fp8(x8, sx, w8, sw, bias=None, batch_bias=None, residual=None, mode=L.CONV_S1, out=None, tile_cfg=12, col_stats_out=None, bias_images=1):
@@ -345,7 +366,7 @@
     B, H, W, _ = x.shape
     Ho, Wo = conv_out_hw(H, W, mode)
     if out is None:
-        out = torch.empty(B, Ho, Wo, w.shape[0], device=x.device, dtype=BF16)
+        out = torch.empty(B, Ho, Wo, w.shape[1] if mode == L.CONV_UP2F else w.shape[0], device=x.device, dtype=BF16)
     d = make_conv_desc(x, w, out, bias, batch_bias, residual, mode, tile_cfg, col_stats_out=col_stats_out, shortcut=shortcut)
     L.check(lib.tmix_conv3x3_nhwc(C.byref(d), _stream()), "tmix_conv3x3_nhwc")
     return out
diff --git a/tweediemix_amd/unet.py b/tweediemix_amd/unet.py
--- a/tweediemix_amd/unet.py
+++ b/tweediemix_amd/unet.py
@@ -115,6 +115,8 @@
                 continue
             if v.dim() == 4 and v.shape[-1] == 3:
                 t[name] = bf(v.to(dev).permute(0, 2, 3, 1))
+                if ".upsamplers." in name:
+                    t[name + ".up2f"] = ops.fold_up2_weight(v.to(dev).permute(0, 2, 3, 1))
             elif v.dim() == 4:
                 t[name] = bf(v.to(dev).reshape(v.shape[0], v.shape[1]))
             elif v.dim() == 2 and ".attn" not in name and ".ff.net.0.proj" not in name:
@@ -639,6 +641,9 @@
             self.op_meta[len(self.ops) - 1] = ("conv_fp8", fl, d)
             return out
         w, bias, sc, csc = self.W[wname + ".weight"], self.W[wname + ".bias"], None, 0
+        taps = 9
+        if mode == L.CONV_UP2 and ops.up2_fold_ok(Hh, Ww):
+            mode, w, taps = L.CONV_UP2F, self.W[wname + ".weight.up2f"], 4
         if shortcut is not None:
             w, bias = self.W.conv2_with_shortcut(shortcut[0])
             sc = (shortcut[1], shortcut[2])
@@ -650,7 +655,7 @@
         self.keep.append(d)
         self._hint_weights(w)
         self._emit(self.lib.tmix_conv3x3_nhwc, C.byref(d))
-        fl = 2 * self.B * Ho * Wo * Cout * (9 * Cin + csc)
+        fl = 2 * self.B * Ho * Wo * Cout * (taps * Cin + csc)
         self.flops += fl
         self.launches["conv"].append((d, fl))
         self._tunable.append((len(self.ops) - 1, "conv", d))
@@ -1082,7 +1087,7 @@
     for p in plans:
         for _i, kind, d in p._tunable:
             k = p._tune_key(kind, d)
-            fl = 2.0 * d.M * d.N * d.K * d.batch if kind == "gemm" else 2.0 * d.B * d.H * d.W * d.Cout * (9 * d.Cin + d.S1_channels + d.S2_channels)
+            fl = 2.0 * d.M * d.N * d.K * d.batch if kind == "gemm" else 2.0 * d.B * d.H * d.W * d.Cout * ((4 if d.mode == L.CONV_UP2F else 9) * d.Cin + d.S1_channels + d.S2_channels)
             weight[k] = weight.get(k, 0.0) + fl
             members.setdefault(k, []).append((p, kind, d))
     base = timed()
diff --git a/tweediemix_amd/vae.py b/tweediemix_amd/vae.py
--- a/tweediemix_amd/vae.py
+++ b/tweediemix_amd/vae.py
@@ -127,6 +127,8 @@
                 t[k] = v.to(F32).contiguous()
             elif v.dim() == 4 and v.shape[-1] == 3 and not k.startswith("decoder.conv_in"):
                 t[k] = v.permute(0, 2, 3, 1).to(BF16).contiguous()
+                if ".upsamplers." in k and ops.up2_fold_enabled():
+                    t[k + ".up2f"] = ops.fold_up2_weight(v.permute(0, 2, 3, 1))
             elif v.dim() == 4 and v.shape[-1] == 1 and not k.startswith("post_quant"):
                 t[k] = v.reshape(v.shape[0], v.shape[1]).to(BF16).contiguous()
             elif v.dim() == 2:
@@ -156,11 +158,14 @@
     def _conv(self, x, name, Hh, Ww, Ci, Co, mode=L.CONV_S1, residual=None):
         Ho, Wo = ops.conv_out_hw(Hh, Ww, mode)
         out = self.arena.get(self.B, Ho * Wo, Co)
-        d = ops.make_conv_desc(x.view(self.B, Hh, Ww, Ci), self.t[name + ".weight"], out.view(self.B, Ho, Wo, Co),
+        w, taps = self.t[name + ".weight"], 9
+        if mode == L.CONV_UP2 and residual is None and ops.up2_fold_ok(Hh, Ww):
+            mode, w, taps = L.CONV_UP2F, self.t[name + ".weight.up2f"], 4
+        d = ops.make_conv_desc(x.view(self.B, Hh, Ww, Ci), w, out.view(self.B, Ho, Wo, Co),
                                self.t[name + ".bias"], None, residual, mode)
         self.keep.append(d)
         self._emit(self.lib.tmix_conv3x3_nhwc, C.byref(d))
-        self.flops += 2 * self.B * Ho * Wo * Co * 9 * Ci
+        self.flops += 2 * self.B * Ho * Wo * Co * taps * Ci
         return out
 
     def _gemm(self, a, w, out, **kw):
```

After: 33.50, median of 6. +1.2%, better.
